# csulb-datascience/TTS-with-Diffusion-model

Measured on NVIDIA B200. Metric: codec_tokens_per_sec, higher is better.
Workload: dtype bf16

## Files before the change

### include/vb200.h

```cpp
#ifndef VB200_H_
#define VB200_H_

#include <stddef.h>
#include <stdint.h>

#ifdef __cplusplus
extern "C" {
#endif

typedef void* vb200_stream_t;

typedef enum {
  VB200_OK = 0,
  VB200_ERR_INVALID = -1,
  VB200_ERR_CUDA = -2,
  VB200_ERR_UNSUPPORTED = -3
} vb200_status;

typedef enum { VB200_F32 = 0, VB200_BF16 = 1, VB200_F16 = 2 } vb200_dtype;

typedef enum {
  VB200_EPI_NONE = 0,
  VB200_EPI_BIAS = 1,
  VB200_EPI_BIAS_GELU = 2,
  VB200_EPI_BIAS_RESIDUAL = 3
} vb200_epilogue;

typedef enum { VB200_ABSORBING = 0, VB200_UNIFORM = 1 } vb200_transition;

typedef enum {
  VB200_NOISE_PHILOX = 0,
  VB200_NOISE_UNIFORMS = 1,
  VB200_NOISE_GREEDY = 2
} vb200_noise;

enum {
  VB200_U_ROW0 = 0,
  VB200_U_TTXT = 1,
  VB200_U_TPROM = 2,
  VB200_U_TRESP = 3,
  VB200_U_TXT0 = 4,
  VB200_U_PROM0 = 5,
  VB200_U_RESP0 = 6,
  VB200_U_GID = 7,
  VB200_U_STRIDE = 8
};

const char* vb200_last_error(void);
int vb200_version(void);
int vb200_device_sms(void);

int vb200_embed_gather(float* x_out, const void* text_w, const void* prom_w, const void* resp_w,
                       const void* sep, const void* time_w, const float* pe,
                       const int32_t* text_ids, const int32_t* prom_ids, const int32_t* resp_ids,
                       const int32_t* utt, const int32_t* row_utt, const int32_t* t_utt,
                       int32_t M, int32_t d, int32_t K, int32_t resp_levels_in,
                       vb200_stream_t stream);


int vb200_adaln(void* out, vb200_dtype out_dtype, const float* x, const float* table, const int32_t* level_utt,
                const int32_t* row_utt, int32_t M, int32_t d, float eps, float k, float c,
                vb200_stream_t stream);

int vb200_layernorm(void* out, vb200_dtype out_dtype, const float* x, const float* weight, const float* bias,
                    int32_t M, int32_t d, float eps, vb200_stream_t stream);

int vb200_gather_rows_bf16(void* out, vb200_dtype out_dtype, const float* x, const int32_t* row_index,
                           int32_t n_rows, int32_t d, vb200_stream_t stream);

int vb200_gemm_bf16(void* out, vb200_dtype out_dtype, const void* A, vb200_dtype a_dtype, const void* W,
                    const float* bias, const float* residual, int32_t M, int32_t N, int32_t K,
                    vb200_epilogue epi, vb200_stream_t stream);

int vb200_gemm_bf16_simt(void* out, vb200_dtype out_dtype, const void* A, vb200_dtype a_dtype, const void* W,
                         const float* bias, const float* residual, int32_t M, int32_t N,
                         int32_t K, vb200_epilogue epi, vb200_stream_t stream);

int vb200_flash_attn_varlen(void* out_bf16, const void* qkv_bf16, const int32_t* cu_rows,
                            int32_t B, int32_t max_T, int32_t M, int32_t n_heads, float scale,
                            vb200_stream_t stream);
int vb200_attn_varlen_simt(void* out_bf16, const void* qkv_bf16, const int32_t* cu_rows,
                           int32_t B, int32_t max_T, int32_t M, int32_t n_heads, float scale,
                           vb200_stream_t stream);

enum {
  VB200_TAB_ONE_KEEP = 0,
  VB200_TAB_ONE_OFF = 1,
  VB200_TAB_ONE_ABSORB = 2,
  VB200_TAB_ONE_BOTH = 3,
  VB200_TAB_CUM_KEEP = 4,
  VB200_TAB_CUM_OFF = 5,
  VB200_TAB_CUM_ABSORB = 6,
  VB200_TAB_CUM_BOTH = 7,
  VB200_TAB_LOG_KEEP = 8,
  VB200_TAB_LOG_OFF = 9,
  VB200_TAB_LOG_ABSORB = 10,
  VB200_TAB_LOG_BOTH = 11,
  VB200_TAB_STRIDE = 12
};

int vb200_q_sample(int32_t* x_out, const int32_t* x0, const int32_t* t_tok, const int32_t* mask,
                   const float* uniforms, const float* table, int32_t n_tok, int32_t K,
                   int32_t S, vb200_transition tr, vb200_stream_t stream);

int vb200_q_sample_dense(int32_t* x_out, const int32_t* x0, const int32_t* t_tok, const int32_t* mask,
                         const float* uniforms, const void* log_qbar_f16, int32_t n_tok, int32_t K,
                         int32_t S, vb200_stream_t stream);

int vb200_q_sample_philox(int32_t* x_out, const int32_t* x0, const int32_t* t_tok, const int32_t* mask,
                          const float* table, int32_t n_tok, int32_t K, int32_t S,
                          vb200_transition tr, uint64_t seed, vb200_stream_t stream);

int vb200_posterior_sample_from_logits(int32_t* x_out, float* post_out, const void* logits,
                                       vb200_dtype logits_dtype, int64_t ld_logits,
                                       const int32_t* x_t, const int32_t* row_utt,
                                       const int32_t* t_utt, const int32_t* utt,
                                       const float* table, int32_t n_rows, int32_t n_levels,
                                       int32_t K, int32_t S, vb200_transition tr,
                                       vb200_noise noise, const float* uniforms, uint64_t seed,
                                       vb200_stream_t stream);

int vb200_head_posterior_sample(int32_t* x_out, void* logits, vb200_dtype logits_dtype,
                                const void* head_in, vb200_dtype head_in_dtype, const void* W,
                                const float* bias, int32_t n_rows, int32_t d, int32_t n_levels, int32_t K,
                                const int32_t* x_t, const int32_t* row_utt, const int32_t* t_utt,
                                const int32_t* utt, const float* table, int32_t S,
                                vb200_transition tr, vb200_noise noise, const float* uniforms,
                                uint64_t seed, vb200_stream_t stream);

int vb200_head_ce_loss(float* loss, const void* head_in, vb200_dtype head_in_dtype, const void* W,
                       const float* bias,
                       const int32_t* targets, int32_t n_rows, int32_t d, int32_t n_levels, int32_t K,
                       vb200_stream_t stream);

int64_t vb200_workspace_bytes(int64_t M, int64_t M_resp, int32_t d, int32_t n_out,
                              vb200_dtype logits_dtype, int64_t* sizes);

int vb200_codes_to_bqt(int64_t* out, const int32_t* codes, const int32_t* utt, int32_t B,
                       int32_t n_levels, int32_t T_max, int64_t pad, vb200_stream_t stream);

int vb200_step_timesteps(int32_t* t_utt, int32_t B, int32_t delta, vb200_stream_t stream);

#ifdef __cplusplus
}
#endif
#endif
```

### tts-with-diffusion-model_b200/csrc/attn_tcgen05.cu

```cuda
#include "common.cuh"
#include <type_traits>

namespace vb200 {

namespace attn {
constexpr int BQ = 128, BKV = 128, HD = 64, KV_STAGES = 2;
constexpr int TILE_BYTES = 128 * HD * 2;
constexpr uint32_t TMEM_COLS = 256;
constexpr uint32_t COL_S = 0, COL_P = 128, COL_O = 192;
constexpr int SOFTMAX_WARPS = 8;
constexpr int THREADS = (SOFTMAX_WARPS + 2) * 32;
constexpr int SMEM_BYTES = TILE_BYTES * (1 + 2 * KV_STAGES) + 1024 + 256;
constexpr float RESCALE_LOG2 = 8.0f;
}

__device__ __forceinline__ void tmem_ld_16x2_x64(uint32_t taddr, uint32_t (&r)[64]) {
  asm volatile(
      "tcgen05.ld.sync.aligned.16x32bx2.x64.b32 "
      "{%0,%1,%2,%3,%4,%5,%6,%7,%8,%9,%10,%11,%12,%13,%14,%15,"
      "%16,%17,%18,%19,%20,%21,%22,%23,%24,%25,%26,%27,%28,%29,%30,%31,"
      "%32,%33,%34,%35,%36,%37,%38,%39,%40,%41,%42,%43,%44,%45,%46,%47,"
      "%48,%49,%50,%51,%52,%53,%54,%55,%56,%57,%58,%59,%60,%61,%62,%63}, [%64], 64;"
      : "=r"(r[0]), "=r"(r[1]), "=r"(r[2]), "=r"(r[3]), "=r"(r[4]), "=r"(r[5]), "=r"(r[6]), "=r"(r[7]),
        "=r"(r[8]), "=r"(r[9]), "=r"(r[10]), "=r"(r[11]), "=r"(r[12]), "=r"(r[13]), "=r"(r[14]), "=r"(r[15]),
        "=r"(r[16]), "=r"(r[17]), "=r"(r[18]), "=r"(r[19]), "=r"(r[20]), "=r"(r[21]), "=r"(r[22]), "=r"(r[23]),
        "=r"(r[24]), "=r"(r[25]), "=r"(r[26]), "=r"(r[27]), "=r"(r[28]), "=r"(r[29]), "=r"(r[30]), "=r"(r[31]),
        "=r"(r[32]), "=r"(r[33]), "=r"(r[34]), "=r"(r[35]), "=r"(r[36]), "=r"(r[37]), "=r"(r[38]), "=r"(r[39]),
        "=r"(r[40]), "=r"(r[41]), "=r"(r[42]), "=r"(r[43]), "=r"(r[44]), "=r"(r[45]), "=r"(r[46]), "=r"(r[47]),
        "=r"(r[48]), "=r"(r[49]), "=r"(r[50]), "=r"(r[51]), "=r"(r[52]), "=r"(r[53]), "=r"(r[54]), "=r"(r[55]),
        "=r"(r[56]), "=r"(r[57]), "=r"(r[58]), "=r"(r[59]), "=r"(r[60]), "=r"(r[61]), "=r"(r[62]), "=r"(r[63])
      : "r"(taddr)
      : "memory");
}
__device__ __forceinline__ void tmem_st_16x2_x32(uint32_t taddr, const uint32_t (&r)[64]) {
  asm volatile(
      "tcgen05.st.sync.aligned.16x32bx2.x32.b32 [%0], 32, "
      "{%1,%2,%3,%4,%5,%6,%7,%8,%9,%10,%11,%12,%13,%14,%15,%16,"
      "%17,%18,%19,%20,%21,%22,%23,%24,%25,%26,%27,%28,%29,%30,%31,%32};"
      ::"r"(taddr), "r"(r[0]), "r"(r[1]), "r"(r[2]), "r"(r[3]), "r"(r[4]), "r"(r[5]), "r"(r[6]), "r"(r[7]),
        "r"(r[8]), "r"(r[9]), "r"(r[10]), "r"(r[11]), "r"(r[12]), "r"(r[13]), "r"(r[14]), "r"(r[15]),
        "r"(r[16]), "r"(r[17]), "r"(r[18]), "r"(r[19]), "r"(r[20]), "r"(r[21]), "r"(r[22]), "r"(r[23]),
        "r"(r[24]), "r"(r[25]), "r"(r[26]), "r"(r[27]), "r"(r[28]), "r"(r[29]), "r"(r[30]), "r"(r[31])
      : "memory");
}
__device__ __forceinline__ void tmem_ld_16x2_x16(uint32_t taddr, uint32_t (&r)[16]) {
  asm volatile(
      "tcgen05.ld.sync.aligned.16x32bx2.x16.b32 "
      "{%0,%1,%2,%3,%4,%5,%6,%7,%8,%9,%10,%11,%12,%13,%14,%15}, [%16], 16;"
      : "=r"(r[0]), "=r"(r[1]), "=r"(r[2]), "=r"(r[3]), "=r"(r[4]), "=r"(r[5]), "=r"(r[6]), "=r"(r[7]),
        "=r"(r[8]), "=r"(r[9]), "=r"(r[10]), "=r"(r[11]), "=r"(r[12]), "=r"(r[13]), "=r"(r[14]), "=r"(r[15])
      : "r"(taddr)
      : "memory");
}
__device__ __forceinline__ void tmem_st_16x2_x16(uint32_t taddr, const uint32_t (&r)[16]) {
  asm volatile(
      "tcgen05.st.sync.aligned.16x32bx2.x16.b32 [%0], 16, "
      "{%1,%2,%3,%4,%5,%6,%7,%8,%9,%10,%11,%12,%13,%14,%15,%16};"
      ::"r"(taddr), "r"(r[0]), "r"(r[1]), "r"(r[2]), "r"(r[3]), "r"(r[4]), "r"(r[5]), "r"(r[6]), "r"(r[7]),
        "r"(r[8]), "r"(r[9]), "r"(r[10]), "r"(r[11]), "r"(r[12]), "r"(r[13]), "r"(r[14]), "r"(r[15])
      : "memory");
}
__device__ __forceinline__ void tmem_st_16x2_x8(uint32_t taddr, const uint32_t (&r)[8]) {
  asm volatile(
      "tcgen05.st.sync.aligned.16x32bx2.x8.b32 [%0], 8, {%1,%2,%3,%4,%5,%6,%7,%8};"
      ::"r"(taddr), "r"(r[0]), "r"(r[1]), "r"(r[2]), "r"(r[3]), "r"(r[4]), "r"(r[5]), "r"(r[6]), "r"(r[7])
      : "memory");
}
__device__ __forceinline__ void tmem_ld_16x2_x32(uint32_t taddr, uint32_t (&r)[32]) {
  asm volatile(
      "tcgen05.ld.sync.aligned.16x32bx2.x32.b32 "
      "{%0,%1,%2,%3,%4,%5,%6,%7,%8,%9,%10,%11,%12,%13,%14,%15,"
      "%16,%17,%18,%19,%20,%21,%22,%23,%24,%25,%26,%27,%28,%29,%30,%31}, [%32], 32;"
      : "=r"(r[0]), "=r"(r[1]), "=r"(r[2]), "=r"(r[3]), "=r"(r[4]), "=r"(r[5]), "=r"(r[6]), "=r"(r[7]),
        "=r"(r[8]), "=r"(r[9]), "=r"(r[10]), "=r"(r[11]), "=r"(r[12]), "=r"(r[13]), "=r"(r[14]), "=r"(r[15]),
        "=r"(r[16]), "=r"(r[17]), "=r"(r[18]), "=r"(r[19]), "=r"(r[20]), "=r"(r[21]), "=r"(r[22]), "=r"(r[23]),
        "=r"(r[24]), "=r"(r[25]), "=r"(r[26]), "=r"(r[27]), "=r"(r[28]), "=r"(r[29]), "=r"(r[30]), "=r"(r[31])
      : "r"(taddr)
      : "memory");
}

__device__ __forceinline__ float ex2_approx(float x) {
  float y;
  asm("ex2.approx.ftz.f32 %0, %1;" : "=f"(y) : "f"(x));
  return y;
}

__device__ __forceinline__ void ex2_poly2(uint64_t x, float& p0, float& p1) {
  float x0, x1;
  unpack2(x, x0, x1);
  x = pack2(fmaxf(x0, -126.0f), fmaxf(x1, -126.0f));
  const uint64_t t = fadd2(x, pack2(12582912.0f, 12582912.0f));
  const uint64_t u = fadd2(t, pack2(-12582912.0f, -12582912.0f));
  const uint64_t r = ffma2(u, pack2(-1.0f, -1.0f), x);
  uint64_t p = ffma2(r, pack2(0.05517167f, 0.05517167f), pack2(0.24261113f, 0.24261113f));
  p = ffma2(r, p, pack2(0.69326097f, 0.69326097f));
  p = ffma2(r, p, pack2(0.99992806f, 0.99992806f));
  float t0, t1, q0, q1;
  unpack2(t, t0, t1);
  unpack2(p, q0, q1);
  p0 = __int_as_float(__float_as_int(q0) + (__float_as_int(t0) << 23));
  p1 = __int_as_float(__float_as_int(q1) + (__float_as_int(t1) << 23));
}
#ifndef VB200_ATTN_EMU_PAIRS
#define VB200_ATTN_EMU_PAIRS 4
#endif
#ifndef VB200_ATTN_EXP_CHUNK
#define VB200_ATTN_EXP_CHUNK 4
#endif
namespace attn { constexpr int EXP_CHUNK = VB200_ATTN_EXP_CHUNK; }

#ifdef VB200_ATTN_TRACE
constexpr int TRACE_CTAS = 1024, TRACE_BLOCKS = 16, TRACE_EVENTS = 8;
__device__ unsigned long long g_attn_trace[TRACE_CTAS * 2 * TRACE_BLOCKS * TRACE_EVENTS];
#define VB_TR(slot, j, ev)                                                                               \
  do {                                                                                                   \
    if (lane == 0 && cta_lin < TRACE_CTAS && (j) < TRACE_BLOCKS)                                         \
      g_attn_trace[((cta_lin * 2 + (slot)) * TRACE_BLOCKS + (j)) * TRACE_EVENTS + (ev)] = clock64();     \
  } while (0)
#else
#define VB_TR(slot, j, ev) do {} while (0)
#endif

__global__ void __launch_bounds__(attn::THREADS, 2) flash_attn_kernel(
    const __grid_constant__ CUtensorMap tm_qkv, __nv_bfloat16* __restrict__ out,
    const int32_t* __restrict__ cu_rows, int n_heads, float scale_log2, float opaque_zero) {
  using namespace attn;
  const int b = blockIdx.z, h = blockIdx.y, qt = blockIdx.x;
  const int row0 = cu_rows[b];
  const int T = cu_rows[b + 1] - row0;
  if (qt * BQ >= T) return;
  const int nblk = (T + BKV - 1) / BKV;
  const int last_valid = T - (nblk - 1) * BKV;
  const int last_n = (last_valid + 15) & ~15;
  const int d = n_heads * HD;

  extern __shared__ uint8_t smem_raw[];
  const uint32_t raw_addr = smem_u32(smem_raw);
  uint8_t* smem = smem_raw + (((raw_addr + 1023u) & ~1023u) - raw_addr);
  uint8_t* s_q = smem;
  uint8_t* s_k = smem + TILE_BYTES;
  uint8_t* s_v = s_k + KV_STAGES * TILE_BYTES;
  uint64_t* bars = reinterpret_cast<uint64_t*>(s_v + KV_STAGES * TILE_BYTES);
  uint64_t* q_full = bars;
  uint64_t* k_full = bars + 1;
  uint64_t* k_empty = k_full + KV_STAGES;
  uint64_t* v_full = k_empty + KV_STAGES;
  uint64_t* v_empty = v_full + KV_STAGES;
  uint64_t* s_full = v_empty + KV_STAGES;
  uint64_t* s_free = s_full + 1;
  uint64_t* p_full = s_free + 1;
  uint64_t* pv_done = p_full + 1;
  uint32_t* tmem_slot = reinterpret_cast<uint32_t*>(pv_done + 1);

  const int warp = __shfl_sync(0xffffffffu, threadIdx.x >> 5, 0);
  const int lane = threadIdx.x & 31;
#ifdef VB200_ATTN_TRACE
  const int cta_lin = blockIdx.x + gridDim.x * (blockIdx.y + gridDim.y * blockIdx.z);
  if (threadIdx.x == 0 && cta_lin < TRACE_CTAS) {
    uint32_t smid;
    asm volatile("mov.u32 %0, %%smid;" : "=r"(smid));
    g_attn_trace[((cta_lin * 2 + 1) * TRACE_BLOCKS + TRACE_BLOCKS - 1) * TRACE_EVENTS + 7] = smid;
    g_attn_trace[((cta_lin * 2 + 1) * TRACE_BLOCKS + TRACE_BLOCKS - 1) * TRACE_EVENTS + 6] = clock64();
  }
#endif

  if (threadIdx.x == SOFTMAX_WARPS * 32) {
    tma_prefetch_desc(&tm_qkv);
    mbar_init(q_full, 1);
    for (int s = 0; s < KV_STAGES; ++s) {
      mbar_init(&k_full[s], 1); mbar_init(&k_empty[s], 1); mbar_init(&v_full[s], 1); mbar_init(&v_empty[s], 1);
    }
    mbar_init(s_full, 1); mbar_init(s_free, SOFTMAX_WARPS); mbar_init(p_full, SOFTMAX_WARPS); mbar_init(pv_done, 1);
    fence_barrier_init();
    pdl_launch_dependents();
    pdl_wait();
    mbar_arrive_expect_tx(q_full, TILE_BYTES);
    tma_load_2d(s_q, &tm_qkv, q_full, h * HD, row0 + qt * BQ);
    mbar_arrive_expect_tx(&k_full[0], TILE_BYTES);
    tma_load_2d(s_k, &tm_qkv, &k_full[0], d + h * HD, row0);
    mbar_arrive_expect_tx(&v_full[0], TILE_BYTES);
    tma_load_2d(s_v, &tm_qkv, &v_full[0], 2 * d + h * HD, row0);
  }
  if (warp == SOFTMAX_WARPS + 1) {
    tmem_alloc(tmem_slot, TMEM_COLS);
    tmem_relinquish();
  }
  tc_fence_before();
  __syncthreads();
  tc_fence_after();
  const uint32_t tmem_base = *tmem_slot;
  pdl_launch_dependents();
  pdl_wait();

  if (warp == SOFTMAX_WARPS) {
    const bool leader = elect_one();
    for (int j = 1; j < nblk; ++j) {
      const int s = j % KV_STAGES;
      const uint32_t ph = (j / KV_STAGES) & 1;
      mbar_wait(&k_empty[s], ph ^ 1);
      if (leader) {
        mbar_arrive_expect_tx(&k_full[s], TILE_BYTES);
        tma_load_2d(s_k + s * TILE_BYTES, &tm_qkv, &k_full[s], d + h * HD, row0 + j * BKV);
      }
      __syncwarp();
      mbar_wait(&v_empty[s], ph ^ 1);
      if (leader) {
        mbar_arrive_expect_tx(&v_full[s], TILE_BYTES);
        tma_load_2d(s_v + s * TILE_BYTES, &tm_qkv, &v_full[s], 2 * d + h * HD, row0 + j * BKV);
      }
      __syncwarp();
    }
  } else if (warp == SOFTMAX_WARPS + 1) {
    const bool leader = elect_one();
    const uint32_t idesc_o = umma_idesc_bf16(BQ, HD, false, true);
    const uint32_t idesc_s_full = umma_idesc_bf16(BQ, BKV, false, false);
    const uint32_t idesc_s_last = umma_idesc_bf16(BQ, last_n, false, false);
    const uint64_t dq = umma_desc_kmajor_sw128(smem_u32(s_q));
    const uint64_t dk_base = umma_desc_kmajor_sw128(smem_u32(s_k));
    const uint64_t dv_base = umma_desc_mnmajor_sw128(smem_u32(s_v), 1024);
    constexpr uint32_t kTileStep = TILE_BYTES >> 4;
    const uint32_t t_s = tmem_base + COL_S, t_p = tmem_base + COL_P, t_o = tmem_base + COL_O;
    auto issue_s = [&](int j) {
      const int st = j % KV_STAGES;
      const uint64_t dk = dk_base + static_cast<uint32_t>(st) * kTileStep;
      const uint32_t idesc_s = (j == nblk - 1) ? idesc_s_last : idesc_s_full;
      if (leader) {
#pragma unroll
        for (int k = 0; k < HD / 16; ++k) umma_ss(t_s, dq + 2 * k, dk + 2 * k, idesc_s, k != 0);
        umma_commit(s_full);
        umma_commit(&k_empty[st]);
      }
      __syncwarp();
    };
    auto issue_pv = [&](int j) {
      const int st = j % KV_STAGES;
      const uint64_t dv = dv_base + static_cast<uint32_t>(st) * kTileStep;
      const uint32_t acc0 = j != 0;
      if (leader) {
        if (j != nblk - 1) {
#pragma unroll
          for (int k = 0; k < BKV / 16; ++k)
            umma_ts(t_o, t_p + k * 8, dv + k * 128, idesc_o, acc0 | (k != 0));
        } else {
          const int ksteps = last_n / 16;
          for (int k = 0; k < ksteps; ++k) umma_ts(t_o, t_p + k * 8, dv + k * 128, idesc_o, acc0 | (k != 0));
        }
        umma_commit(pv_done);
        umma_commit(&v_empty[st]);
      }
      __syncwarp();
    };
    mbar_wait(q_full, 0);
    mbar_wait(&k_full[0], 0);
    tc_fence_after();
    issue_s(0);
    for (int j = 0; j < nblk; ++j) {
      if (j + 1 < nblk) {
        mbar_wait(&k_full[(j + 1) % KV_STAGES], ((j + 1) / KV_STAGES) & 1);
        mbar_wait(s_free, j & 1);
        tc_fence_after();
        VB_TR(1, j, 0);
        issue_s(j + 1);
      }
      mbar_wait(&v_full[j % KV_STAGES], (j / KV_STAGES) & 1);
      mbar_wait(p_full, j & 1);
      tc_fence_after();
      VB_TR(1, j, 1);
      issue_pv(j);
    }
  } else {
    const int quad = warp & 3;
    const int half_rows = warp >> 2;
    const int t0 = lane & 15, t1 = lane >> 4;
    const int r_tile = quad * 32 + half_rows * 16 + t0;
    const uint32_t t_x = tmem_base + (static_cast<uint32_t>(quad * 32 + half_rows * 16) << 16);
    if (qt * BQ + quad * 32 + half_rows * 16 >= T) {
      for (int j = 0; j < nblk; ++j) {
        mbar_wait(s_full, j & 1);
        if (lane == 0) mbar_arrive(s_free);
        if (j > 0) mbar_wait(pv_done, (j - 1) & 1);
        if (lane == 0) mbar_arrive(p_full);
      }
      mbar_wait(pv_done, (nblk - 1) & 1);
    } else {
      float m_ref = -INFINITY, l = 0.f;
      const uint64_t zero2 = pack2(opaque_zero, opaque_zero);
      auto move_reference = [&](float bm, int j) {
        if (j == 0) {
          m_ref = bm;
          return;
        }
        const bool grow = (bm - m_ref) * scale_log2 > RESCALE_LOG2;
        if (__any_sync(0xffffffffu, grow)) {
          const float m_new = grow ? bm : m_ref;
          const float alpha = ex2_approx((m_ref - m_new) * scale_log2);
          m_ref = m_new;
          l *= alpha;
          mbar_wait(pv_done, (j - 1) & 1);
          tc_fence_after();
#pragma unroll 1
          for (int c = 0; c < 2; ++c) {
            uint32_t o[16];
            tmem_ld_16x2_x16(t_x + COL_O + c * 32, o);
            tmem_ld_wait();
#pragma unroll
            for (int i = 0; i < 16; ++i) o[i] = __float_as_uint(__uint_as_float(o[i]) * alpha);
            tmem_st_16x2_x16(t_x + COL_O + c * 32, o);
          }
        }
      };
      auto key_block = [&](int j, auto tail_tag) {
        constexpr bool tail = decltype(tail_tag)::value;
        if (warp == 0) VB_TR(0, j, 0);
        mbar_wait(s_full, j & 1);
        tc_fence_after();
        if (warp == 0) VB_TR(0, j, 1);
        uint32_t s[64];
        tmem_ld_16x2_x64(t_x + COL_S, s);
        tmem_ld_wait();
        if (warp == 0) VB_TR(0, j, 2);
        tc_fence_before();
        __syncwarp();
        if (lane == 0) mbar_arrive(s_free);
        if (tail) {
#pragma unroll
          for (int i = 0; i < 64; ++i)
            if (t1 * 64 + i >= last_valid) s[i] = __float_as_uint(-INFINITY);
        }
        float bm0 = -INFINITY, bm1 = -INFINITY, bm2 = -INFINITY, bm3 = -INFINITY;
#pragma unroll
        for (int i = 0; i < 64; i += 4) {
          bm0 = fmaxf(bm0, __uint_as_float(s[i]));     bm1 = fmaxf(bm1, __uint_as_float(s[i + 1]));
          bm2 = fmaxf(bm2, __uint_as_float(s[i + 2])); bm3 = fmaxf(bm3, __uint_as_float(s[i + 3]));
        }
        float bm = fmaxf(fmaxf(bm0, bm1), fmaxf(bm2, bm3));
        bm = fmaxf(bm, __shfl_xor_sync(0xffffffffu, bm, 16));
        move_reference(bm, j);
        const float mneg = -m_ref * scale_log2;
#ifdef VB200_ATTN_TRACE
        if (warp == 0 && mneg != 12345.f) VB_TR(0, j, 3);
#endif
        const uint64_t scale2 = pack2(scale_log2, scale_log2), mneg2 = pack2(mneg, mneg);
        uint64_t ps[2] = {0ull, 0ull};
#pragma unroll
        for (int k = 0; k < 32 / EXP_CHUNK; ++k) {
          const uint64_t mn2 = k >= 2 ? ffma2(ps[k & 1], zero2, mneg2) : mneg2;
#pragma unroll
          for (int i = k * EXP_CHUNK; i < (k + 1) * EXP_CHUNK; ++i) {
            const uint64_t x = ffma2(pack2(__uint_as_float(s[2 * i]), __uint_as_float(s[2 * i + 1])), scale2, mn2);
            const int ii = i & 15;
            const bool emulate = ((ii + 1) * VB200_ATTN_EMU_PAIRS) / 16 != (ii * VB200_ATTN_EMU_PAIRS) / 16;
            float p0, p1;
            if (emulate) {
              ex2_poly2(x, p0, p1);
            } else {
              float x0, x1;
              unpack2(x, x0, x1);
              p0 = ex2_approx(x0);
              p1 = ex2_approx(x1);
            }
            ps[k & 1] = fadd2(ps[k & 1], pack2(p0, p1));
            s[i] = pack_bf16x2(p0, p1);
          }
        }
        float a0, a1, a2, a3;
        unpack2(ps[0], a0, a1);
        unpack2(ps[1], a2, a3);
        l += (a0 + a1) + (a2 + a3);
#ifdef VB200_ATTN_TRACE
        if (warp == 0 && l != -1.f) VB_TR(0, j, 4);
#endif
        if (j > 0) {
          mbar_wait(pv_done, (j - 1) & 1);
          tc_fence_after();
        }
        if (warp == 0) VB_TR(0, j, 5);
        tmem_st_16x2_x32(t_x + COL_P, s);
        tmem_st_wait();
        tc_fence_before();
        __syncwarp();
        if (lane == 0) mbar_arrive(p_full);
        if (warp == 0) VB_TR(0, j, 6);
      };
      auto short_block = [&](int j) {
        mbar_wait(s_full, j & 1);
        tc_fence_after();
        uint32_t sq[16];
        tmem_ld_16x2_x16(t_x + COL_S, sq);
        tmem_ld_wait();
        tc_fence_before();
        __syncwarp();
        if (lane == 0) mbar_arrive(s_free);
        float bm = -INFINITY;
#pragma unroll
        for (int i = 0; i < 16; ++i) {
          if (t1 * 16 + i >= last_valid) sq[i] = __float_as_uint(-INFINITY);
          bm = fmaxf(bm, __uint_as_float(sq[i]));
        }
        bm = fmaxf(bm, __shfl_xor_sync(0xffffffffu, bm, 16));
        move_reference(bm, j);
        const float mneg = -m_ref * scale_log2;
        uint32_t pq[8];
#pragma unroll
        for (int i = 0; i < 8; ++i) {
          const float p0 = ex2_approx(fmaf(__uint_as_float(sq[2 * i]), scale_log2, mneg));
          const float p1 = ex2_approx(fmaf(__uint_as_float(sq[2 * i + 1]), scale_log2, mneg));
          l += p0 + p1;
          pq[i] = pack_bf16x2(p0, p1);
        }
        if (j > 0) {
          mbar_wait(pv_done, (j - 1) & 1);
          tc_fence_after();
        }
        tmem_st_16x2_x8(t_x + COL_P, pq);
        tmem_st_wait();
        tc_fence_before();
        __syncwarp();
        if (lane == 0) mbar_arrive(p_full);
      };
      const int n_full = last_valid < BKV ? nblk - 1 : nblk;
#pragma unroll 1
      for (int j = 0; j < n_full; ++j) key_block(j, std::false_type{});
      if (n_full < nblk) {
        if (last_valid <= 32) short_block(n_full);
        else key_block(n_full, std::true_type{});
      }
      mbar_wait(pv_done, (nblk - 1) & 1);
      tc_fence_after();
      l += __shfl_xor_sync(0xffffffffu, l, 16);
      uint32_t o[32];
      tmem_ld_16x2_x32(t_x + COL_O, o);
      tmem_ld_wait();
      const int q_row = qt * BQ + r_tile;
      if (q_row < T) {
        const float inv = 1.0f / l;
        __nv_bfloat16* o_dst = out + static_cast<size_t>(row0 + q_row) * d + h * HD + t1 * 32;
#pragma unroll
        for (int i = 0; i < 32; i += 8) {
          uint4 pk;
          pk.x = pack_bf16x2(__uint_as_float(o[i]) * inv, __uint_as_float(o[i + 1]) * inv);
          pk.y = pack_bf16x2(__uint_as_float(o[i + 2]) * inv, __uint_as_float(o[i + 3]) * inv);
          pk.z = pack_bf16x2(__uint_as_float(o[i + 4]) * inv, __uint_as_float(o[i + 5]) * inv);
          pk.w = pack_bf16x2(__uint_as_float(o[i + 6]) * inv, __uint_as_float(o[i + 7]) * inv);
          *reinterpret_cast<uint4*>(o_dst + i) = pk;
        }
      }
    }
  }

  tc_fence_before();
  __syncthreads();
  if (warp == SOFTMAX_WARPS + 1) {
    __syncwarp();
    tc_fence_after();
    tmem_dealloc(tmem_base, TMEM_COLS);
  }
}

}

using namespace vb200;

#ifdef VB200_ATTN_TRACE
extern "C" int vb200_debug_attn_trace(unsigned long long* host_dst, size_t n_words) {
  const size_t n = sizeof(g_attn_trace) / sizeof(unsigned long long);
  cudaError_t e = cudaMemcpyFromSymbol(host_dst, g_attn_trace, (n_words < n ? n_words : n) * sizeof(unsigned long long));
  return e == cudaSuccess ? 0 : -1;
}
#endif

extern "C" int vb200_flash_attn_varlen(void* out_bf16, const void* qkv_bf16, const int32_t* cu_rows,
                                       int32_t B, int32_t max_T, int32_t M, int32_t n_heads,
                                       float scale, vb200_stream_t stream) {
  using namespace attn;
  if (M == 0) return VB200_OK;
  VB_REQUIRE(out_bf16 && qkv_bf16 && cu_rows, "flash_attn: null pointer");
  VB_REQUIRE(B >= 1 && B <= 65535 && n_heads >= 1 && n_heads <= 65535 && max_T >= 1 && M >= 0,
             "flash_attn: bad sizes B=%d heads=%d max_T=%d M=%d", B, n_heads, max_T, M);
  const int d = n_heads * HD;
  CUtensorMap tm;
  int rc = cached_tmap(&tm, VB200_BF16, qkv_bf16, static_cast<uint64_t>(3) * d, M,
                       static_cast<uint64_t>(3) * d * 2, HD, 128);
  if (rc != VB200_OK) return rc;
  dim3 grid((max_T + BQ - 1) / BQ, n_heads, B);
  const float sl2 = scale * 1.4426950408889634f;
  constexpr int SMEM_SOLO = 116 * 1024;
  const bool solo = static_cast<long long>(grid.x) * grid.y * grid.z <= num_sms();
  const int smem_bytes = solo ? SMEM_SOLO : SMEM_BYTES;
  VB_CONFIGURE_SMEM(flash_attn_kernel, SMEM_SOLO);
  {
    static std::atomic<uint64_t> carveout_done{0};
    int dev = 0;
    VB_CHECK_CUDA(cudaGetDevice(&dev));
    const uint64_t bit = 1ull << (dev & 63);
    if (!(carveout_done.load(std::memory_order_acquire) & bit)) {
      VB_CHECK_CUDA(cudaFuncSetAttribute(flash_attn_kernel, cudaFuncAttributePreferredSharedMemoryCarveout,
                                         cudaSharedmemCarveoutMaxShared));
      carveout_done.fetch_or(bit, std::memory_order_release);
    }
  }
  PdlTag pdl_tag(solo ? 16 : 64);
  VB_CHECK_CUDA(launch_pdl(flash_attn_kernel, grid, dim3(THREADS), smem_bytes, static_cast<cudaStream_t>(stream), 1,
                           tm, static_cast<__nv_bfloat16*>(out_bf16), cu_rows, n_heads, sl2, 0.0f));
  VB_CHECK_CUDA(cudaGetLastError());
  return VB200_OK;
}
```

### tts-with-diffusion-model_b200/csrc/common.cuh

```cuda
#pragma once
#include <atomic>
#include <cuda.h>
#include <cuda_bf16.h>
#include <cuda_fp16.h>
#include <cuda_runtime.h>
#include <stdint.h>

#include "../../include/vb200.h"

namespace vb200 {

void set_error(const char* fmt, ...);
int cuda_fail(cudaError_t e, const char* what);
#define VB_CHECK_CUDA(expr)                                              \
  do {                                                                   \
    cudaError_t _e = (expr);                                             \
    if (_e != cudaSuccess) return ::vb200::cuda_fail(_e, #expr);         \
  } while (0)
#define VB_REQUIRE(cond, ...)                                            \
  do {                                                                   \
    if (!(cond)) {                                                       \
      ::vb200::set_error(__VA_ARGS__);                                   \
      return VB200_ERR_INVALID;                                          \
    }                                                                    \
  } while (0)

int num_sms();

bool head_sample_supported(int d, int K, int noise);
int head_sample_fused(int32_t* x_out, const void* head_in, const void* W, const float* bias, const int32_t* x_t,
                      const int32_t* row_utt, const int32_t* t_utt, const int32_t* utt, const float* table,
                      int n_rows, int d, int n_levels, int K, int S, int tr, int noise, uint64_t seed,
                      int in_f16, cudaStream_t st);
int head_ce_fused(float* loss_out, const void* head_in, const void* W, const float* bias, const int32_t* targets,
                  int n_rows, int d, int n_levels, int K, int in_f16, cudaStream_t st);

#define VB_CONFIGURE_SMEM(kern, bytes)                                                                   \
  do {                                                                                                   \
    static std::atomic<uint64_t> vb_cfg_done{0};                                                         \
    int vb_cfg_dev = 0;                                                                                  \
    VB_CHECK_CUDA(cudaGetDevice(&vb_cfg_dev));                                                           \
    const uint64_t vb_cfg_bit = 1ull << (vb_cfg_dev & 63);                                               \
    if (!(vb_cfg_done.load(std::memory_order_acquire) & vb_cfg_bit)) {                                   \
      VB_CHECK_CUDA(cudaFuncSetAttribute(kern, cudaFuncAttributeMaxDynamicSharedMemorySize, bytes));     \
      vb_cfg_done.fetch_or(vb_cfg_bit, std::memory_order_release);                                       \
    }                                                                                                    \
  } while (0)
bool pdl_enabled();
int pdl_mask();
extern thread_local int g_pdl_tag;
struct PdlTag {
  int prev;
  explicit PdlTag(int t) : prev(g_pdl_tag) { g_pdl_tag = t; }
  ~PdlTag() { g_pdl_tag = prev; }
};
template <typename... KArgs, typename... Args>
inline cudaError_t launch_pdl(void (*kern)(KArgs...), dim3 grid, dim3 block, size_t smem, cudaStream_t st,
                              int cluster_x, Args&&... args) {
  cudaLaunchConfig_t cfg = {};
  cfg.gridDim = grid;
  cfg.blockDim = block;
  cfg.dynamicSmemBytes = smem;
  cfg.stream = st;
  cudaLaunchAttribute attr[2];
  int n = 0;
  if (cluster_x > 1) {
    attr[n].id = cudaLaunchAttributeClusterDimension;
    attr[n].val.clusterDim.x = cluster_x;
    attr[n].val.clusterDim.y = 1;
    attr[n].val.clusterDim.z = 1;
    ++n;
  }
  if (pdl_mask() & (1 | g_pdl_tag)) {
    attr[n].id = cudaLaunchAttributeProgrammaticStreamSerialization;
    attr[n].val.programmaticStreamSerializationAllowed = 1;
    ++n;
  }
  cfg.attrs = attr;
  cfg.numAttrs = n;
  return cudaLaunchKernelEx(&cfg, kern, static_cast<KArgs>(args)...);
}

int make_tmap_2d(CUtensorMap* out, vb200_dtype dtype, const void* gptr, uint64_t inner,
                 uint64_t outer, uint64_t row_stride_bytes, uint32_t box_inner, uint32_t box_outer);
int cached_tmap(CUtensorMap* out, vb200_dtype dtype, const void* ptr, uint64_t inner,
                uint64_t outer, uint64_t stride_bytes, uint32_t box_inner, uint32_t box_outer);

__device__ __forceinline__ void pdl_launch_dependents() { asm volatile("griddepcontrol.launch_dependents;"); }
__device__ __forceinline__ void pdl_wait() { asm volatile("griddepcontrol.wait;" ::: "memory"); }

#ifdef __CUDACC__

__device__ __forceinline__ uint32_t smem_u32(const void* p) {
  return static_cast<uint32_t>(__cvta_generic_to_shared(p));
}

__device__ __forceinline__ bool elect_one() {
  uint32_t pred = 0;
  asm volatile(
      "{\n\t.reg .pred P;\n\t"
      "elect.sync _|P, 0xffffffff;\n\t"
      "selp.b32 %0, 1, 0, P;\n\t}"
      : "=r"(pred));
  return pred != 0;
}

__device__ __forceinline__ void mbar_init(uint64_t* bar, uint32_t count) {
  asm volatile("mbarrier.init.shared::cta.b64 [%0], %1;" ::"r"(smem_u32(bar)), "r"(count));
}
__device__ __forceinline__ void fence_barrier_init() {
  asm volatile("fence.mbarrier_init.release.cluster;" ::: "memory");
}
__device__ __forceinline__ void fence_proxy_async_smem() {
  asm volatile("fence.proxy.async.shared::cta;" ::: "memory");
}
__device__ __forceinline__ void mbar_arrive_expect_tx(uint64_t* bar, uint32_t bytes) {
  asm volatile("mbarrier.arrive.expect_tx.shared::cta.b64 _, [%0], %1;" ::"r"(smem_u32(bar)),
               "r"(bytes)
               : "memory");
}
__device__ __forceinline__ void mbar_arrive(uint64_t* bar) {
  asm volatile("mbarrier.arrive.shared::cta.b64 _, [%0];" ::"r"(smem_u32(bar)) : "memory");
}
__device__ __forceinline__ bool mbar_try_wait(uint64_t* bar, uint32_t parity) {
  uint32_t ok;
  asm volatile(
      "{\n\t.reg .pred P;\n\t"
      "mbarrier.try_wait.parity.shared::cta.b64 P, [%1], %2;\n\t"
      "selp.b32 %0, 1, 0, P;\n\t}"
      : "=r"(ok)
      : "r"(smem_u32(bar)), "r"(parity)
      : "memory");
  return ok != 0;
}
__device__ __forceinline__ bool mbar_test_wait(uint64_t* bar, uint32_t parity) {
  uint32_t ok;
  asm volatile(
      "{\n\t.reg .pred P;\n\t"
      "mbarrier.test_wait.parity.shared::cta.b64 P, [%1], %2;\n\t"
      "selp.b32 %0, 1, 0, P;\n\t}"
      : "=r"(ok)
      : "r"(smem_u32(bar)), "r"(parity)
      : "memory");
  return ok != 0;
}
__device__ __forceinline__ void mbar_wait(uint64_t* bar, uint32_t parity) {
  uint32_t spins = 0;
  while (!mbar_try_wait(bar, parity)) {
    if (++spins > (1u << 24)) __trap();
  }
}

__device__ __forceinline__ void prefetch_l1(const void* p) {
  asm volatile("prefetch.global.L1 [%0];" ::"l"(p));
}
__device__ __forceinline__ void tma_prefetch_desc(const CUtensorMap* m) {
  asm volatile("prefetch.tensormap [%0];" ::"l"(reinterpret_cast<uint64_t>(m)) : "memory");
}
__device__ __forceinline__ void tma_load_2d(void* smem_dst, const CUtensorMap* m, uint64_t* bar,
                                            int32_t c_inner, int32_t c_outer) {
  asm volatile(
      "cp.async.bulk.tensor.2d.shared::cluster.global.mbarrier::complete_tx::bytes"
      " [%0], [%1, {%3, %4}], [%2];"
      ::"r"(smem_u32(smem_dst)), "l"(reinterpret_cast<uint64_t>(m)), "r"(smem_u32(bar)),
      "r"(c_inner), "r"(c_outer)
      : "memory");
}

__device__ __forceinline__ void tma_store_2d(const CUtensorMap* m, const void* smem_src,
                                             int32_t c_inner, int32_t c_outer) {
  asm volatile("cp.async.bulk.tensor.2d.global.shared::cta.bulk_group [%0, {%2, %3}], [%1];"
               ::"l"(reinterpret_cast<uint64_t>(m)), "r"(smem_u32(smem_src)), "r"(c_inner),
               "r"(c_outer)
               : "memory");
}
__device__ __forceinline__ void tma_reduce_add_2d(const CUtensorMap* m, const void* smem_src,
                                                  int32_t c_inner, int32_t c_outer) {
  asm volatile("cp.reduce.async.bulk.tensor.2d.global.shared::cta.add.bulk_group [%0, {%2, %3}], [%1];"
               ::"l"(reinterpret_cast<uint64_t>(m)), "r"(smem_u32(smem_src)), "r"(c_inner),
               "r"(c_outer)
               : "memory");
}
__device__ __forceinline__ void tma_store_commit() {
  asm volatile("cp.async.bulk.commit_group;" ::: "memory");
}
__device__ __forceinline__ void tma_store_wait_read() {
  asm volatile("cp.async.bulk.wait_group.read 0;" ::: "memory");
}
__device__ __forceinline__ void tma_store_wait_all() {
  asm volatile("cp.async.bulk.wait_group 0;" ::: "memory");
}

__device__ __forceinline__ void tmem_alloc(uint32_t* smem_slot, uint32_t ncols) {
  asm volatile("tcgen05.alloc.cta_group::1.sync.aligned.shared::cta.b32 [%0], %1;" ::"r"(
                   smem_u32(smem_slot)),
               "r"(ncols)
               : "memory");
}
__device__ __forceinline__ void tmem_relinquish() {
  asm volatile("tcgen05.relinquish_alloc_permit.cta_group::1.sync.aligned;" ::: "memory");
}
__device__ __forceinline__ void tmem_dealloc(uint32_t taddr, uint32_t ncols) {
  asm volatile("tcgen05.dealloc.cta_group::1.sync.aligned.b32 %0, %1;" ::"r"(taddr), "r"(ncols)
               : "memory");
}
__device__ __forceinline__ void tc_fence_before() {
  asm volatile("tcgen05.fence::before_thread_sync;" ::: "memory");
}
__device__ __forceinline__ void tc_fence_after() {
  asm volatile("tcgen05.fence::after_thread_sync;" ::: "memory");
}
__device__ __forceinline__ void umma_ss(uint32_t tmem_d, uint64_t desc_a, uint64_t desc_b,
                                        uint32_t idesc, uint32_t accumulate) {
  asm volatile(
      "{\n\t.reg .pred p;\n\t"
      "setp.ne.b32 p, %4, 0;\n\t"
      "tcgen05.mma.cta_group::1.kind::f16 [%0], %1, %2, %3, p;\n\t}"
      ::"r"(tmem_d), "l"(desc_a), "l"(desc_b), "r"(idesc), "r"(accumulate)
      : "memory");
}
__device__ __forceinline__ void umma_ts(uint32_t tmem_d, uint32_t tmem_a, uint64_t desc_b,
                                        uint32_t idesc, uint32_t accumulate) {
  asm volatile(
      "{\n\t.reg .pred p;\n\t"
      "setp.ne.b32 p, %4, 0;\n\t"
      "tcgen05.mma.cta_group::1.kind::f16 [%0], [%1], %2, %3, p;\n\t}"
      ::"r"(tmem_d), "r"(tmem_a), "l"(desc_b), "r"(idesc), "r"(accumulate)
      : "memory");
}
__device__ __forceinline__ void umma_commit(uint64_t* bar) {
  asm volatile("tcgen05.commit.cta_group::1.mbarrier::arrive::one.shared::cluster.b64 [%0];" ::"r"(
                   smem_u32(bar))
               : "memory");
}
__device__ __forceinline__ void tmem_ld_wait() {
  asm volatile("tcgen05.wait::ld.sync.aligned;" ::: "memory");
}
__device__ __forceinline__ void tmem_st_wait() {
  asm volatile("tcgen05.wait::st.sync.aligned;" ::: "memory");
}
__device__ __forceinline__ void tmem_ld_32x32(uint32_t taddr, uint32_t (&r)[32]) {
  asm volatile(
      "tcgen05.ld.sync.aligned.32x32b.x32.b32 "
      "{%0,%1,%2,%3,%4,%5,%6,%7,%8,%9,%10,%11,%12,%13,%14,%15,"
      "%16,%17,%18,%19,%20,%21,%22,%23,%24,%25,%26,%27,%28,%29,%30,%31}, [%32];"
      : "=r"(r[0]), "=r"(r[1]), "=r"(r[2]), "=r"(r[3]), "=r"(r[4]), "=r"(r[5]), "=r"(r[6]),
        "=r"(r[7]), "=r"(r[8]), "=r"(r[9]), "=r"(r[10]), "=r"(r[11]), "=r"(r[12]), "=r"(r[13]),
        "=r"(r[14]), "=r"(r[15]), "=r"(r[16]), "=r"(r[17]), "=r"(r[18]), "=r"(r[19]),
        "=r"(r[20]), "=r"(r[21]), "=r"(r[22]), "=r"(r[23]), "=r"(r[24]), "=r"(r[25]),
        "=r"(r[26]), "=r"(r[27]), "=r"(r[28]), "=r"(r[29]), "=r"(r[30]), "=r"(r[31])
      : "r"(taddr)
      : "memory");
}
__device__ __forceinline__ void tmem_st_32x32(uint32_t taddr, const uint32_t (&r)[32]) {
  asm volatile(
      "tcgen05.st.sync.aligned.32x32b.x32.b32 [%0], "
      "{%1,%2,%3,%4,%5,%6,%7,%8,%9,%10,%11,%12,%13,%14,%15,%16,"
      "%17,%18,%19,%20,%21,%22,%23,%24,%25,%26,%27,%28,%29,%30,%31,%32};"
      ::"r"(taddr), "r"(r[0]), "r"(r[1]), "r"(r[2]), "r"(r[3]), "r"(r[4]), "r"(r[5]), "r"(r[6]),
      "r"(r[7]), "r"(r[8]), "r"(r[9]), "r"(r[10]), "r"(r[11]), "r"(r[12]), "r"(r[13]),
      "r"(r[14]), "r"(r[15]), "r"(r[16]), "r"(r[17]), "r"(r[18]), "r"(r[19]), "r"(r[20]),
      "r"(r[21]), "r"(r[22]), "r"(r[23]), "r"(r[24]), "r"(r[25]), "r"(r[26]), "r"(r[27]),
      "r"(r[28]), "r"(r[29]), "r"(r[30]), "r"(r[31])
      : "memory");
}

__device__ __forceinline__ uint32_t cluster_ctarank() {
  uint32_t r;
  asm volatile("mov.u32 %0, %%cluster_ctarank;" : "=r"(r));
  return r;
}
__device__ __forceinline__ void cluster_sync_all() {
  asm volatile("barrier.cluster.arrive.release.aligned;" ::: "memory");
  asm volatile("barrier.cluster.wait.acquire.aligned;" ::: "memory");
}
__device__ __forceinline__ void tma_load_2d_pair(void* smem_dst, const CUtensorMap* m, uint64_t* bar,
                                                 int32_t c_inner, int32_t c_outer) {
  asm volatile(
      "cp.async.bulk.tensor.2d.cta_group::2.shared::cluster.global.mbarrier::complete_tx::bytes"
      " [%0], [%1, {%3, %4}], [%2];"
      ::"r"(smem_u32(smem_dst)), "l"(reinterpret_cast<uint64_t>(m)), "r"(smem_u32(bar) & 0xFEFFFFFFu),
      "r"(c_inner), "r"(c_outer)
      : "memory");
}
__device__ __forceinline__ void tmem_alloc_pair(uint32_t* smem_slot, uint32_t ncols) {
  asm volatile("tcgen05.alloc.cta_group::2.sync.aligned.shared::cta.b32 [%0], %1;" ::"r"(
                   smem_u32(smem_slot)),
               "r"(ncols)
               : "memory");
}
__device__ __forceinline__ void tmem_relinquish_pair() {
  asm volatile("tcgen05.relinquish_alloc_permit.cta_group::2.sync.aligned;" ::: "memory");
}
__device__ __forceinline__ void tmem_dealloc_pair(uint32_t taddr, uint32_t ncols) {
  asm volatile("tcgen05.dealloc.cta_group::2.sync.aligned.b32 %0, %1;" ::"r"(taddr), "r"(ncols)
               : "memory");
}
__device__ __forceinline__ void umma_ss_pair(uint32_t tmem_d, uint64_t desc_a, uint64_t desc_b,
                                             uint32_t idesc, uint32_t accumulate) {
  asm volatile(
      "{\n\t.reg .pred p;\n\t"
      "setp.ne.b32 p, %4, 0;\n\t"
      "tcgen05.mma.cta_group::2.kind::f16 [%0], %1, %2, %3, p;\n\t}"
      ::"r"(tmem_d), "l"(desc_a), "l"(desc_b), "r"(idesc), "r"(accumulate)
      : "memory");
}
__device__ __forceinline__ void umma_commit_pair(uint64_t* bar) {
  const uint16_t mask = 3;
  asm volatile(
      "tcgen05.commit.cta_group::2.mbarrier::arrive::one.shared::cluster.multicast::cluster.b64 [%0], %1;"
      ::"r"(smem_u32(bar)), "h"(mask)
      : "memory");
}
__device__ __forceinline__ void mbar_arrive_remote(uint64_t* bar, uint32_t rank) {
  uint32_t remote;
  asm volatile("mapa.shared::cluster.u32 %0, %1, %2;" : "=r"(remote) : "r"(smem_u32(bar)), "r"(rank));
  asm volatile("mbarrier.arrive.release.cluster.shared::cluster.b64 _, [%0];" ::"r"(remote) : "memory");
}

__device__ __forceinline__ uint64_t umma_desc_kmajor_sw128(uint32_t smem_addr) {
  uint64_t d = 0;
  d |= static_cast<uint64_t>((smem_addr & 0x3FFFF) >> 4);
  d |= static_cast<uint64_t>(1) << 16;
  d |= static_cast<uint64_t>(1024 >> 4) << 32;
  d |= static_cast<uint64_t>(1) << 46;
  d |= static_cast<uint64_t>(2) << 61;
  return d;
}
__device__ __forceinline__ uint64_t umma_desc_mnmajor_sw128(uint32_t smem_addr, uint32_t lbo_bytes) {
  uint64_t d = 0;
  d |= static_cast<uint64_t>((smem_addr & 0x3FFFF) >> 4);
  d |= static_cast<uint64_t>((lbo_bytes >> 4) & 0x3FFF) << 16;
  d |= static_cast<uint64_t>(1024 >> 4) << 32;
  d |= static_cast<uint64_t>(1) << 46;
  d |= static_cast<uint64_t>(2) << 61;
  return d;
}
constexpr uint32_t kIdescBf16 = (1u << 7) | (1u << 10);
__host__ __device__ constexpr uint32_t umma_idesc_bf16(uint32_t M, uint32_t N, bool a_mn_major,
                                                       bool b_mn_major) {
  return (1u << 4)
         | kIdescBf16
         | ((a_mn_major ? 1u : 0u) << 15)
         | ((b_mn_major ? 1u : 0u) << 16)
         | ((N >> 3) << 17)
         | ((M >> 4) << 24);
}

__device__ __forceinline__ uint32_t pack_bf16x2(float lo, float hi) {
  __nv_bfloat162 v = __floats2bfloat162_rn(lo, hi);
  return *reinterpret_cast<uint32_t*>(&v);
}
__device__ __forceinline__ uint32_t pack_f16x2(float lo, float hi) {
  uint32_t v;
  asm("cvt.rn.satfinite.f16x2.f32 %0, %1, %2;" : "=r"(v) : "f"(hi), "f"(lo));
  return v;
}
__device__ __forceinline__ uint32_t pack_act16x2(float lo, float hi, bool f16) {
  return f16 ? pack_f16x2(lo, hi) : pack_bf16x2(lo, hi);
}

__device__ __forceinline__ uint64_t pack2(float lo, float hi) {
  uint64_t r;
  asm("mov.b64 %0, {%1, %2};" : "=l"(r) : "f"(lo), "f"(hi));
  return r;
}
__device__ __forceinline__ void unpack2(uint64_t v, float& lo, float& hi) {
  asm("mov.b64 {%0, %1}, %2;" : "=f"(lo), "=f"(hi) : "l"(v));
}
__device__ __forceinline__ uint64_t ffma2(uint64_t a, uint64_t b, uint64_t c) {
  uint64_t d;
  asm("fma.rn.f32x2 %0, %1, %2, %3;" : "=l"(d) : "l"(a), "l"(b), "l"(c));
  return d;
}
__device__ __forceinline__ uint64_t fadd2(uint64_t a, uint64_t b) {
  uint64_t d;
  asm("add.rn.f32x2 %0, %1, %2;" : "=l"(d) : "l"(a), "l"(b));
  return d;
}
constexpr float kEps = 1.0e-6f;

struct Philox {
  uint32_t k0, k1;
  __device__ __forceinline__ uint4 operator()(uint32_t c0, uint32_t c1, uint32_t c2, uint32_t c3) const {
    uint32_t a = k0, b = k1;
#pragma unroll
    for (int r = 0; r < 10; ++r) {
      const uint32_t hi0 = __umulhi(0xD2511F53u, c0), lo0 = 0xD2511F53u * c0;
      const uint32_t hi1 = __umulhi(0xCD9E8D57u, c2), lo1 = 0xCD9E8D57u * c2;
      c0 = hi1 ^ c1 ^ a;
      c1 = lo1;
      c2 = hi0 ^ c3 ^ b;
      c3 = lo0;
      a += 0x9E3779B9u;
      b += 0xBB67AE85u;
    }
    return make_uint4(c0, c1, c2, c3);
  }
};
__device__ __forceinline__ float u01(uint32_t x) { return (x >> 8) * 5.9604644775390625e-8f; }
__device__ __forceinline__ float exp2f_fast(float x) {
  float y;
  asm("ex2.approx.ftz.f32 %0, %1;" : "=f"(y) : "f"(x));
  return y;
}

__device__ __forceinline__ float warp_sum(float v) {
#pragma unroll
  for (int o = 16; o > 0; o >>= 1) v += __shfl_xor_sync(0xffffffffu, v, o);
  return v;
}
__device__ __forceinline__ float warp_max(float v) {
#pragma unroll
  for (int o = 16; o > 0; o >>= 1) v = fmaxf(v, __shfl_xor_sync(0xffffffffu, v, o));
  return v;
}

#endif

template <int NV>
__device__ __forceinline__ void adaln_row_finish(const float (&v)[NV][8], const float (&g)[NV][8],
                                                 const float (&bt)[NV][8], __nv_bfloat16* orow, int lane,
                                                 float eps, float k, float c, bool f16 = false) {
  constexpr int d = NV * 256;
  float s = 0.f;
#pragma unroll
  for (int i = 0; i < NV; ++i)
#pragma unroll
    for (int e = 0; e < 8; ++e) s += v[i][e];
  const float mean = warp_sum(s) * (1.0f / d);
  float q = 0.f;
#pragma unroll
  for (int i = 0; i < NV; ++i)
#pragma unroll
    for (int e = 0; e < 8; ++e) { const float dv = v[i][e] - mean; q += dv * dv; }
  const float rstd = rsqrtf(warp_sum(q) * (1.0f / d) + eps);
#pragma unroll
  for (int i = 0; i < NV; ++i) {
    float y[8];
#pragma unroll
    for (int e = 0; e < 8; ++e) {
      float h = (v[i][e] - mean) * rstd;
      h = c * (1.f - k * h) * h;
      y[e] = fmaf(g[i][e], h, bt[i][e]);
    }
    uint4 o;
    o.x = pack_act16x2(y[0], y[1], f16); o.y = pack_act16x2(y[2], y[3], f16);
    o.z = pack_act16x2(y[4], y[5], f16); o.w = pack_act16x2(y[6], y[7], f16);
    *reinterpret_cast<uint4*>(orow + i * 256 + lane * 8) = o;
  }
}
template <int NV>
__device__ __forceinline__ void adaln_load_params(const float* __restrict__ table, int lvl, int lane,
                                                  float (&g)[NV][8], float (&bt)[NV][8]) {
  constexpr int d = NV * 256;
  const float* gp = table + static_cast<size_t>(lvl) * 2 * d;
#pragma unroll
  for (int i = 0; i < NV; ++i) {
    const float4 g0 = __ldg(reinterpret_cast<const float4*>(gp + i * 256 + lane * 8));
    const float4 g1 = __ldg(reinterpret_cast<const float4*>(gp + i * 256 + lane * 8 + 4));
    const float4 b0 = __ldg(reinterpret_cast<const float4*>(gp + d + i * 256 + lane * 8));
    const float4 b1 = __ldg(reinterpret_cast<const float4*>(gp + d + i * 256 + lane * 8 + 4));
    g[i][0] = g0.x; g[i][1] = g0.y; g[i][2] = g0.z; g[i][3] = g0.w;
    g[i][4] = g1.x; g[i][5] = g1.y; g[i][6] = g1.z; g[i][7] = g1.w;
    bt[i][0] = b0.x; bt[i][1] = b0.y; bt[i][2] = b0.z; bt[i][3] = b0.w;
    bt[i][4] = b1.x; bt[i][5] = b1.y; bt[i][6] = b1.z; bt[i][7] = b1.w;
  }
}

}
```

### tts-with-diffusion-model_b200/csrc/gemm_tcgen05.cu

```cuda
#include <stdlib.h>

#include <type_traits>

#include "common.cuh"

#ifndef VB200_GEMM_BIAS_PREFETCH
#define VB200_GEMM_BIAS_PREFETCH 1
#endif
#ifndef VB200_GEMM_EARLY_LOAD
#define VB200_GEMM_EARLY_LOAD 1
#endif

namespace vb200 {

namespace gemm {
constexpr int BM = 128, BK = 64;
constexpr int A_BYTES = BM * BK * 2;
template <int CTAS, int BN> struct Cfg {
  static constexpr int B_ROWS = BN / CTAS;
  static constexpr int B_BYTES = B_ROWS * BK * 2;
  static constexpr int STAGE_BYTES = A_BYTES + B_BYTES;
  static constexpr int STAGES = (4 * 48 * 1024) / STAGE_BYTES;
};
constexpr int EPI_WARPS = 8;
constexpr int THREADS = (2 + EPI_WARPS) * 32;
constexpr int EPI_TILE_BYTES = 32 * 128;
constexpr int SMEM_BYTES = 4 * 48 * 1024 + EPI_WARPS * EPI_TILE_BYTES + 1024  +
                           256 ;
constexpr uint32_t TMEM_COLS = 512;
}

__device__ __forceinline__ void gelu_erf_fast2(float& x0, float& x1) {
  const float z0 = fminf(fabsf(x0) * 0.70710678118654752f, 6.0f);
  const float z1 = fminf(fabsf(x1) * 0.70710678118654752f, 6.0f);
  const uint64_t z = pack2(z0, z1);
  uint64_t p = ffma2(z, pack2(9.22344479e-05f, 9.22344479e-05f), pack2(-2.20238999e-03f, -2.20238999e-03f));
  p = ffma2(z, p, pack2(2.23510694e-02f, 2.23510694e-02f));
  p = ffma2(z, p, pack2(-1.29628107e-01f, -1.29628107e-01f));
  p = ffma2(z, p, pack2(-9.38564420e-01f, -9.38564420e-01f));
  p = ffma2(z, p, pack2(-1.62045550e+00f, -1.62045550e+00f));
  p = ffma2(z, p, pack2(-1.00044155e+00f, -1.00044155e+00f));
  float p0, p1, q0, q1, h0, h1;
  unpack2(p, p0, p1);
  asm("ex2.approx.ftz.f32 %0, %1;" : "=f"(q0) : "f"(p0));
  asm("ex2.approx.ftz.f32 %0, %1;" : "=f"(q1) : "f"(p1));
  unpack2(ffma2(pack2(q0, q1), pack2(-1.0f, -1.0f), pack2(0.5f, 0.5f)), h0, h1);
  h0 = __uint_as_float(__float_as_uint(h0) | (__float_as_uint(x0) & 0x80000000u));
  h1 = __uint_as_float(__float_as_uint(h1) | (__float_as_uint(x1) & 0x80000000u));
  const uint64_t s = fadd2(pack2(h0, h1), pack2(0.5f, 0.5f));
  unpack2(ffma2(pack2(x0, x1), s, 0ull), x0, x1);
}

template <int EPI, typename OutT, int CTAS, int BN>
__global__ void __launch_bounds__(gemm::THREADS, 1) gemm_tcgen05_kernel(
    const __grid_constant__ CUtensorMap tm_a, const __grid_constant__ CUtensorMap tm_b,
    const __grid_constant__ CUtensorMap tm_out, const float* __restrict__ bias, int M, int N, int K,
    uint32_t a_is_f16) {
  using namespace gemm;
  using C = Cfg<CTAS, BN>;
  constexpr int STAGES = C::STAGES, STAGE_BYTES = C::STAGE_BYTES, B_ROWS = C::B_ROWS;
  constexpr int HALF_COLS = BN / 2;
  const uint32_t cta_rank = CTAS == 2 ? cluster_ctarank() : 0;
  extern __shared__ uint8_t smem_raw[];
  const uint32_t raw_addr = smem_u32(smem_raw);
  const uint32_t pad = ((raw_addr + 1023u) & ~1023u) - raw_addr;
  uint8_t* smem = smem_raw + pad;
  uint8_t* epi_smem = smem + STAGES * STAGE_BYTES;
  uint64_t* bars = reinterpret_cast<uint64_t*>(epi_smem + EPI_WARPS * EPI_TILE_BYTES);
  uint64_t* full = bars;
  uint64_t* empty = bars + STAGES;
  uint64_t* acc_full = bars + 2 * STAGES;
  uint64_t* acc_empty = acc_full + 2;
  uint32_t* tmem_slot = reinterpret_cast<uint32_t*>(acc_empty + 2);

  const int warp = __shfl_sync(0xffffffffu, threadIdx.x >> 5, 0);
  const int lane = threadIdx.x & 31;
  const int num_m = (M + BM * CTAS - 1) / (BM * CTAS), num_n = (N + BN - 1) / BN;
  const int num_tiles = num_m * num_n;
  const int num_kb = (K + BK - 1) / BK;
  const int tile0 = blockIdx.x / CTAS, tile_stride = gridDim.x / CTAS;

  if (threadIdx.x == 0) {
    tma_prefetch_desc(&tm_a);
    tma_prefetch_desc(&tm_b);
    tma_prefetch_desc(&tm_out);
    for (int s = 0; s < STAGES; ++s) { mbar_init(&full[s], 1); mbar_init(&empty[s], 1); }
    for (int a = 0; a < 2; ++a) { mbar_init(&acc_full[a], 1); mbar_init(&acc_empty[a], EPI_WARPS * CTAS); }
    fence_barrier_init();
#if VB200_GEMM_EARLY_LOAD
    if (CTAS == 1 && tile0 < num_tiles) {
      pdl_launch_dependents();
      const int m_row = (tile0 / num_n) * BM, n_row = (tile0 % num_n) * BN;
      const int n_pre = num_kb < STAGES ? num_kb : STAGES;
      for (int kb = 0; kb < n_pre; ++kb) {
        mbar_arrive_expect_tx(&full[kb], STAGE_BYTES);
        tma_load_2d(smem + kb * STAGE_BYTES + A_BYTES, &tm_b, &full[kb], kb * BK, n_row);
      }
      pdl_wait();
      for (int kb = 0; kb < n_pre; ++kb) tma_load_2d(smem + kb * STAGE_BYTES, &tm_a, &full[kb], kb * BK, m_row);
    }
#endif
  }
  if (warp == 1) {
    if (CTAS == 2) { tmem_alloc_pair(tmem_slot, TMEM_COLS); tmem_relinquish_pair(); }
    else { tmem_alloc(tmem_slot, TMEM_COLS); tmem_relinquish(); }
  }
  tc_fence_before();
  if (CTAS == 2) cluster_sync_all(); else __syncthreads();
  tc_fence_after();
  const uint32_t tmem_base = *tmem_slot;
  pdl_launch_dependents();
  pdl_wait();

  if (warp == 0) {
    {
      const bool leader = elect_one();
      int stage = 0; uint32_t phase = 0;
      int kb0 = 0;
#if VB200_GEMM_EARLY_LOAD
      if (CTAS == 1) {
        kb0 = num_kb < STAGES ? num_kb : STAGES;
        if (kb0 == STAGES) phase = 1; else stage = kb0;
      }
#endif
      for (int tile = tile0; tile < num_tiles; tile += tile_stride) {
        const int m_blk = tile / num_n, n_blk = tile % num_n;
        const int m_row = (m_blk * CTAS + cta_rank) * BM, n_row = n_blk * BN + cta_rank * B_ROWS;
        for (int kb = kb0; kb < num_kb; ++kb) {
          mbar_wait(&empty[stage], phase ^ 1);
          uint8_t* sa = smem + stage * STAGE_BYTES;
          if (leader) {
            if (CTAS == 2) {
              if (cta_rank == 0) mbar_arrive_expect_tx(&full[stage], 2 * STAGE_BYTES);
              tma_load_2d_pair(sa, &tm_a, &full[stage], kb * BK, m_row);
              tma_load_2d_pair(sa + A_BYTES, &tm_b, &full[stage], kb * BK, n_row);
            } else {
              mbar_arrive_expect_tx(&full[stage], STAGE_BYTES);
              tma_load_2d(sa, &tm_a, &full[stage], kb * BK, m_row);
              tma_load_2d(sa + A_BYTES, &tm_b, &full[stage], kb * BK, n_row);
            }
          }
          __syncwarp();
          if (++stage == STAGES) { stage = 0; phase ^= 1; }
        }
        kb0 = 0;
      }
    }
  } else if (warp == 1) {
    if (cta_rank == 0) {
      const bool leader = elect_one();
      const uint32_t idesc = umma_idesc_bf16(BM * CTAS, BN, false, false) & ~(a_is_f16 ? kIdescBf16 : 0u);
      int stage = 0; uint32_t phase = 0;
      int it = 0;
      for (int tile = tile0; tile < num_tiles; tile += tile_stride, ++it) {
        const int as = it & 1;
        const uint32_t aphase = (it >> 1) & 1;
        mbar_wait(&acc_empty[as], aphase ^ 1);
        tc_fence_after();
        const uint32_t d_tmem = tmem_base + as * BN;
        for (int kb = 0; kb < num_kb; ++kb) {
          mbar_wait(&full[stage], phase);
          tc_fence_after();
          const uint32_t sa = smem_u32(smem + stage * STAGE_BYTES);
          const uint64_t da = umma_desc_kmajor_sw128(sa);
          const uint64_t db = umma_desc_kmajor_sw128(sa + A_BYTES);
          if (leader) {
#pragma unroll
            for (int k = 0; k < BK / 16; ++k) {
              if (CTAS == 2) umma_ss_pair(d_tmem, da + 2 * k, db + 2 * k, idesc, (kb | k) != 0);
              else umma_ss(d_tmem, da + 2 * k, db + 2 * k, idesc, (kb | k) != 0);
            }
            if (CTAS == 2) umma_commit_pair(&empty[stage]);
            else umma_commit(&empty[stage]);
          }
          __syncwarp();
          if (++stage == STAGES) { stage = 0; phase ^= 1; }
        }
        if (leader) {
          if (CTAS == 2) umma_commit_pair(&acc_full[as]); else umma_commit(&acc_full[as]);
        }
        __syncwarp();
      }
    }
  } else {
    const int e = warp - 2;
    const int quad = warp & 3;
    const int half = e >> 2;
    uint8_t* stage_tile = epi_smem + e * EPI_TILE_BYTES;
    uint8_t* my_row = stage_tile + lane * 128;
    const int sw = lane & 7;
    constexpr bool kWide = sizeof(OutT) == 4;
    constexpr int CHUNK_COLS = kWide ? 32 : 64;
    constexpr int HALF0_COLS = BN == 192 ? 128 : HALF_COLS;
    const int col_base = half * HALF0_COLS;
    const int n_chunks = (half == 0 ? HALF0_COLS : BN - HALF0_COLS) / CHUNK_COLS;
    const bool epi_leader = elect_one();
    int it = 0;
    for (int tile = tile0; tile < num_tiles; tile += tile_stride, ++it) {
      const int m_blk = tile / num_n, n_blk = tile % num_n;
      const int as = it & 1;
      const uint32_t aphase = (it >> 1) & 1;
      if (EPI != VB200_EPI_NONE && VB200_GEMM_BIAS_PREFETCH) {
        const int nb0 = n_blk * BN + col_base + lane * 32;
        if (lane * 32 < n_chunks * CHUNK_COLS && nb0 < N) prefetch_l1(bias + nb0);
      }
      mbar_wait(&acc_full[as], aphase);
      tc_fence_after();
      const int row0 = (m_blk * CTAS + cta_rank) * BM + quad * 32;
      const uint32_t t_row = tmem_base + (static_cast<uint32_t>(quad * 32) << 16) + as * BN + col_base;
#pragma unroll 1
      for (int c = 0; c < n_chunks; ++c) {
        const int n0 = n_blk * BN + col_base + c * CHUNK_COLS;
        if (epi_leader) tma_store_wait_read();
        __syncwarp();
#pragma unroll
        for (int sub = 0; sub < CHUNK_COLS / 32; ++sub) {
          uint32_t r[32];
          tmem_ld_32x32(t_row + c * CHUNK_COLS + sub * 32, r);
          tmem_ld_wait();
          float v[32];
#pragma unroll
          for (int i = 0; i < 32; ++i) v[i] = __uint_as_float(r[i]);
          const int nb = n0 + sub * 32;
          if (EPI != VB200_EPI_NONE) {
            if (nb + 32 <= N) {
#pragma unroll
              for (int i = 0; i < 32; i += 4) {
                const float4 b4 = __ldg(reinterpret_cast<const float4*>(bias + nb + i));
                unpack2(fadd2(pack2(v[i], v[i + 1]), pack2(b4.x, b4.y)), v[i], v[i + 1]);
                unpack2(fadd2(pack2(v[i + 2], v[i + 3]), pack2(b4.z, b4.w)), v[i + 2], v[i + 3]);
              }
            } else {
#pragma unroll
              for (int i = 0; i < 32; ++i) if (nb + i < N) v[i] += __ldg(bias + nb + i);
            }
          }
          if (EPI == VB200_EPI_BIAS_GELU) {
#pragma unroll
            for (int i = 0; i < 32; i += 2) gelu_erf_fast2(v[i], v[i + 1]);
          }
          if (kWide) {
#pragma unroll
            for (int q = 0; q < 8; ++q)
              *reinterpret_cast<float4*>(my_row + ((q ^ sw) << 4)) =
                  make_float4(v[4 * q], v[4 * q + 1], v[4 * q + 2], v[4 * q + 3]);
          } else {
            constexpr bool is_bf16 = std::is_same<OutT, __nv_bfloat16>::value;
#pragma unroll
            for (int q = 0; q < 4; ++q) {
              uint4 p;
              if (is_bf16) {
                p.x = pack_bf16x2(v[8 * q], v[8 * q + 1]); p.y = pack_bf16x2(v[8 * q + 2], v[8 * q + 3]);
                p.z = pack_bf16x2(v[8 * q + 4], v[8 * q + 5]); p.w = pack_bf16x2(v[8 * q + 6], v[8 * q + 7]);
              } else {
                p.x = pack_f16x2(v[8 * q], v[8 * q + 1]); p.y = pack_f16x2(v[8 * q + 2], v[8 * q + 3]);
                p.z = pack_f16x2(v[8 * q + 4], v[8 * q + 5]); p.w = pack_f16x2(v[8 * q + 6], v[8 * q + 7]);
              }
              *reinterpret_cast<uint4*>(my_row + (((sub * 4 + q) ^ sw) << 4)) = p;
            }
          }
        }
        fence_proxy_async_smem();
        __syncwarp();
        if (epi_leader && row0 < M && n0 < N) {
          if (EPI == VB200_EPI_BIAS_RESIDUAL) tma_reduce_add_2d(&tm_out, stage_tile, n0, row0);
          else tma_store_2d(&tm_out, stage_tile, n0, row0);
          tma_store_commit();
        }
      }
      tc_fence_before();
      __syncwarp();
      if (lane == 0) {
        if (CTAS == 2 && cta_rank != 0) mbar_arrive_remote(&acc_empty[as], 0);
        else mbar_arrive(&acc_empty[as]);
      }
    }
    if (epi_leader) tma_store_wait_all();
  }

  tc_fence_before();
  if (CTAS == 2) cluster_sync_all(); else __syncthreads();
  if (warp == 1) {
    __syncwarp();
    tc_fence_after();
    if (CTAS == 2) tmem_dealloc_pair(tmem_base, TMEM_COLS); else tmem_dealloc(tmem_base, TMEM_COLS);
  }
}

template <int EPI, typename OutT>
static int launch_gemm(void* out, vb200_dtype dt, const void* A, vb200_dtype a_dt, const void* W, const float* bias,
                       int M, int N, int K, cudaStream_t st) {
  const uint32_t a_f16 = a_dt == VB200_F16 ? 1u : 0u;
  using namespace gemm;
  PdlTag pdl_tag(EPI == VB200_EPI_BIAS_RESIDUAL ? 8 : 4);
  constexpr int BN = 256;
  const int sms = num_sms(), mt = (M + BM - 1) / BM, nn = (N + BN - 1) / BN;
  const long ksteps = static_cast<long>((K + BK - 1) / BK) * (BK / 16);
  auto waves = [](long tiles, long units) { return (tiles + units - 1) / units; };
  const long t_wide = waves(static_cast<long>(mt) * nn, sms) * ksteps * 163;
  const long t_pair = waves(static_cast<long>((M + 2 * BM - 1) / (2 * BM)) * nn, sms / 2) * ksteps * 135 + 5000;
  const long t_narrow = N > 128 ? waves(static_cast<long>(mt) * ((N + 127) / 128), sms) * ksteps * 99 : (1l << 60);
  const long t_n64 = (sizeof(OutT) == 4 && N > 64) ? waves(static_cast<long>(mt) * ((N + 63) / 64), sms) * ksteps * 75
                                                   : (1l << 60);
  const long tiles_192 = static_cast<long>(mt) * (N / 192);
  const long t_n192 = (sizeof(OutT) == 2 && N % 192 == 0 && tiles_192 <= sms) ? ksteps * 130 : (1l << 60);
  int ctas = t_pair <= t_wide ? 2 : 1;
  bool narrow = false, narrow64 = false, n192 = false;
  long best = ctas == 2 ? t_pair : t_wide;
  if (t_narrow < best) { ctas = 1; narrow = true; best = t_narrow; }
  if (t_n64 < best) { ctas = 1; narrow = false; narrow64 = true; best = t_n64; }
  if (t_n192 < best) { ctas = 1; narrow = false; narrow64 = false; n192 = true; best = t_n192; }
  static int tile_forced = -1;
  if (tile_forced < 0) {
    const char* e = getenv("VB200_GEMM_TILE");
    tile_forced = !e ? 0 : e[0] == 'p' ? 1 : e[0] == 'w' ? 2 : (e[0] == 'n' && e[1] == 'a') ? 3 : (e[0] == 'n' && e[1] == '6') ? 4 : 0;
  }
  if (tile_forced) {
    ctas = tile_forced == 1 ? 2 : 1;
    narrow = tile_forced == 3 && N > 128;
    narrow64 = tile_forced == 4 && sizeof(OutT) == 4 && N > 64;
    n192 = false;
  }
  const int bn = n192 ? 192 : narrow64 ? 64 : (narrow ? 128 : BN);
  CUtensorMap ta, tb, tout;
  int rc = cached_tmap(&ta, a_dt, A, K, M, static_cast<uint64_t>(K) * 2, BK, BM);
  if (rc != VB200_OK) return rc;
  rc = cached_tmap(&tb, a_dt, W, K, N, static_cast<uint64_t>(K) * 2, BK, bn / ctas);
  if (rc != VB200_OK) return rc;
  const int esz = sizeof(OutT);
  rc = cached_tmap(&tout, dt, out, N, M, static_cast<uint64_t>(N) * esz, 128 / esz, 32);
  if (rc != VB200_OK) return rc;
  const int tiles = ((M + BM * ctas - 1) / (BM * ctas)) * ((N + bn - 1) / bn);
  const int groups = num_sms() / ctas;
  const int grid = (tiles < groups ? tiles : groups) * ctas;
  if (n192) {
    if constexpr (sizeof(OutT) == 2) {
      auto kern = gemm_tcgen05_kernel<EPI, OutT, 1, 192>;
      VB_CONFIGURE_SMEM(kern, SMEM_BYTES);
      VB_CHECK_CUDA(launch_pdl(kern, dim3(grid), dim3(THREADS), SMEM_BYTES, st, 1, ta, tb, tout, bias, M, N, K, a_f16));
    }
  } else if (narrow64) {
    if constexpr (sizeof(OutT) == 4) {
      auto kern = gemm_tcgen05_kernel<EPI, OutT, 1, 64>;
      VB_CONFIGURE_SMEM(kern, SMEM_BYTES);
      VB_CHECK_CUDA(launch_pdl(kern, dim3(grid), dim3(THREADS), SMEM_BYTES, st, 1, ta, tb, tout, bias, M, N, K, a_f16));
    }
  } else if (narrow) {
    auto kern = gemm_tcgen05_kernel<EPI, OutT, 1, 128>;
    VB_CONFIGURE_SMEM(kern, SMEM_BYTES);
    VB_CHECK_CUDA(launch_pdl(kern, dim3(grid), dim3(THREADS), SMEM_BYTES, st, 1, ta, tb, tout, bias, M, N, K, a_f16));
  } else if (ctas == 1) {
    auto kern = gemm_tcgen05_kernel<EPI, OutT, 1, 256>;
    VB_CONFIGURE_SMEM(kern, SMEM_BYTES);
    VB_CHECK_CUDA(launch_pdl(kern, dim3(grid), dim3(THREADS), SMEM_BYTES, st, 1, ta, tb, tout, bias, M, N, K, a_f16));
  } else {
    auto kern = gemm_tcgen05_kernel<EPI, OutT, 2, 256>;
    VB_CONFIGURE_SMEM(kern, SMEM_BYTES);
    VB_CHECK_CUDA(launch_pdl(kern, dim3(grid), dim3(THREADS), SMEM_BYTES, st, 2, ta, tb, tout, bias, M, N, K, a_f16));
  }
  VB_CHECK_CUDA(cudaGetLastError());
  return VB200_OK;
}

template <int EPI>
static int launch_gemm_dtype(void* out, vb200_dtype dt, const void* A, vb200_dtype a_dt, const void* W,
                             const float* bias, int M, int N, int K, cudaStream_t st) {
  switch (dt) {
    case VB200_F32: return launch_gemm<EPI, float>(out, dt, A, a_dt, W, bias, M, N, K, st);
    case VB200_BF16: return launch_gemm<EPI, __nv_bfloat16>(out, dt, A, a_dt, W, bias, M, N, K, st);
    case VB200_F16: return launch_gemm<EPI, __half>(out, dt, A, a_dt, W, bias, M, N, K, st);
  }
  set_error("gemm: unknown out dtype %d", static_cast<int>(dt));
  return VB200_ERR_INVALID;
}

}

using namespace vb200;

extern "C" int vb200_gemm_bf16(void* out, vb200_dtype out_dtype, const void* A, vb200_dtype a_dtype, const void* W,
                               const float* bias, const float* residual, int32_t M, int32_t N,
                               int32_t K, vb200_epilogue epi, vb200_stream_t stream) {
  VB_REQUIRE(M >= 0 && N > 0 && K > 0, "gemm: bad sizes M=%d N=%d K=%d", M, N, K);
  VB_REQUIRE(a_dtype == VB200_BF16 || a_dtype == VB200_F16, "gemm: A and W must be bf16 or f16");
  if (M == 0) return VB200_OK;
  VB_REQUIRE(out && A && W, "gemm: null pointer");
  VB_REQUIRE(K % 8 == 0, "gemm: K=%d must be a multiple of 8 (TMA row stride is 16-byte granular)", K);
  VB_REQUIRE(N % 8 == 0, "gemm: N=%d must be a multiple of 8 (16-byte vector stores)", N);
  VB_REQUIRE((reinterpret_cast<uintptr_t>(out) & 15) == 0, "gemm: out must be 16-byte aligned");
  VB_REQUIRE(epi == VB200_EPI_NONE || bias, "gemm: epilogue %d needs bias", static_cast<int>(epi));
  VB_REQUIRE(epi != VB200_EPI_BIAS_RESIDUAL || (residual && out_dtype == VB200_F32),
             "gemm: BIAS_RESIDUAL needs residual and fp32 output");
  cudaStream_t st = static_cast<cudaStream_t>(stream);
  switch (epi) {
    case VB200_EPI_NONE: return launch_gemm_dtype<VB200_EPI_NONE>(out, out_dtype, A, a_dtype, W, bias, M, N, K, st);
    case VB200_EPI_BIAS: return launch_gemm_dtype<VB200_EPI_BIAS>(out, out_dtype, A, a_dtype, W, bias, M, N, K, st);
    case VB200_EPI_BIAS_GELU: return launch_gemm_dtype<VB200_EPI_BIAS_GELU>(out, out_dtype, A, a_dtype, W, bias, M, N, K, st);
    case VB200_EPI_BIAS_RESIDUAL:
      if (residual != static_cast<const float*>(out))
        VB_CHECK_CUDA(cudaMemcpyAsync(out, residual, static_cast<size_t>(M) * N * sizeof(float),
                                      cudaMemcpyDeviceToDevice, st));
      return launch_gemm<VB200_EPI_BIAS_RESIDUAL, float>(out, out_dtype, A, a_dtype, W, bias, M, N, K, st);
  }
  set_error("gemm: unknown epilogue %d", static_cast<int>(epi));
  return VB200_ERR_INVALID;
}
```

### tts-with-diffusion-model_b200/vall_e/b200/engine.py

```python
from __future__ import annotations

import math
import os
from dataclasses import dataclass, field

import numpy as np
import torch

from . import lib as L


def sinusoidal_table(n: int, d_model: int) -> torch.Tensor:
    d_half = d_model // 2
    omega = torch.exp(-math.log(1e4) * (torch.arange(d_half, dtype=torch.float32) / d_half))
    ang = omega[None, :] * torch.arange(n)[:, None]
    return torch.cat([ang.sin(), ang.cos()], dim=-1).contiguous()


def _act_dtypes():
    v = os.environ.get("VB200_ACT", "head")
    on = {"h", "ff", "head"} if v == "f16" else (set() if v == "bf16" else {x.strip() for x in v.split(",")})
    if not on <= {"h", "ff", "head"}:
        raise ValueError(f"VB200_ACT={v!r}: expected f16, bf16 or a comma list of h, ff, head")
    return {k: (torch.float16 if k in on else torch.bfloat16) for k in ("h", "ff", "head")}


ACT = _act_dtypes()


class PackedWeights:

    def __init__(self, sd: dict, n_heads: int, n_layers: int, norm_type: str, device, max_rows: int = 4096):
        dev = torch.device(device)
        if dev.type != "cuda":
            raise L.VB200Error("PackedWeights needs a CUDA device (no CPU fallback)")
        bf = lambda t: t.detach().to(dev, torch.bfloat16).contiguous()
        as_ = lambda t, k: t.detach().to(dev, ACT[k]).contiguous()
        f32 = lambda t: t.detach().to(dev, torch.float32).contiguous()
        self.device = dev
        self.n_heads, self.n_layers, self.norm_type = n_heads, n_layers, norm_type
        self.d = int(sd["sep"].shape[0])
        if self.d % n_heads or self.d // n_heads != 64:
            raise L.VB200Error(f"head_dim must be 64 (d_model={self.d}, n_heads={n_heads})")
        self.text_w = bf(sd["text_emb.weight"])
        self.prom_w = bf(sd["proms_emb.weight"])
        self.resp_w = bf(sd["resps_emb.weight"])
        self.K = int(self.prom_w.shape[1])
        if int(self.resp_w.shape[1]) != self.K:
            raise L.VB200Error("resps_emb and proms_emb must have the same number of classes")
        self.sep = bf(sd["sep"])
        self.time_w = bf(sd["time_emb.weight"]) if "time_emb.weight" in sd else None
        self.layers = []
        for i in range(n_layers):
            p = f"blocks.{i}"
            ly = dict(
                w_qkv=as_(sd[f"{p}.attn.block.to_qkv.weight"], "h"),
                w_out=bf(sd[f"{p}.attn.block.to_out.weight"]),
                b_out=f32(sd[f"{p}.attn.block.to_out.bias"]),
                w_ff1=as_(sd[f"{p}.ffn.block.0.weight"], "h"), b_ff1=f32(sd[f"{p}.ffn.block.0.bias"]),
                w_ff2=as_(sd[f"{p}.ffn.block.3.weight"], "ff"), b_ff2=f32(sd[f"{p}.ffn.block.3.bias"]),
            )
            for which in ("attn", "ffn"):
                if norm_type == "adaln":
                    emb = sd[f"{p}.{which}.norm.emb.weight"].detach().float()
                    logg, beta = emb.chunk(2, dim=-1)
                    ly[f"norm_{which}"] = f32(torch.cat([logg.exp(), beta], dim=-1))
                else:
                    ly[f"norm_{which}"] = (f32(sd[f"{p}.{which}.norm.weight"]), f32(sd[f"{p}.{which}.norm.bias"]))
            self.layers.append(ly)
        self.w_cls = as_(sd["classifier.weight"], "head")
        self.b_cls = f32(sd["classifier.bias"])
        self.n_out = int(self.w_cls.shape[0])
        self._pe, self._pe_retired = None, []
        self.ensure_pe(max_rows)

    def ensure_pe(self, n: int) -> torch.Tensor:
        if self._pe is None or self._pe.shape[0] < n:
            if self._pe is not None:
                self._pe_retired.append(self._pe)
            self._pe = sinusoidal_table(max(n, 1), self.d).to(self.device)
        return self._pe


def check_ids(ids: torch.Tensor, n: int, what: str, lo: int = 0) -> None:
    if ids.numel() == 0 or os.environ.get("VB200_CHECK_IDS", "1")[:1] == "0":
        return
    mn, mx = torch.aminmax(ids)
    mn, mx = int(mn), int(mx)
    if mn < lo or mx >= n:
        raise IndexError(f"{what}: ids must lie in [{lo}, {n}), got [{mn}, {mx}]")


class BatchLayout:

    def __init__(self, text_list, proms_list, resp_lens, device, gids=None, n_text: int | None = None,
                 n_codes: int | None = None):
        dev = torch.device(device)
        B = len(text_list)
        if B == 0:
            raise ValueError("empty batch")
        if not (len(proms_list) == B and len(resp_lens) == B):
            raise ValueError("text_list, proms_list and resps must have the same length")
        t_txt = [int(t.shape[0]) for t in text_list]
        t_prom = [int(p.shape[0]) for p in proms_list]
        t_resp = [int(r) for r in resp_lens]
        for p in proms_list:
            if p.dim() != 2 or p.shape[1] != 8:
                raise ValueError(f"prompts must be (t, 8) code grids, got {tuple(p.shape)}")
        rows = [a + 1 + b + 1 + c for a, b, c in zip(t_txt, t_prom, t_resp)]
        cu = np.zeros(B + 1, dtype=np.int64)
        cu[1:] = np.cumsum(rows)
        if cu[-1] >= 2 ** 31:
            raise ValueError("batch too large for int32 row indices")
        self.B, self.M, self.max_T = B, int(cu[-1]), int(max(rows))
        self.t_txt, self.t_prom, self.t_resp, self.rows = t_txt, t_prom, t_resp, rows
        self.M_resp = int(sum(t_resp))
        utt = np.zeros((B, L.U_STRIDE), dtype=np.int32)
        utt[:, L.U_ROW0] = cu[:-1]
        utt[:, L.U_TTXT], utt[:, L.U_TPROM], utt[:, L.U_TRESP] = t_txt, t_prom, t_resp
        utt[:, L.U_TXT0] = np.concatenate([[0], np.cumsum(t_txt)[:-1]])
        utt[:, L.U_PROM0] = np.concatenate([[0], np.cumsum(t_prom)[:-1]])
        resp0 = np.concatenate([[0], np.cumsum(t_resp)[:-1]])
        utt[:, L.U_RESP0] = resp0
        utt[:, L.U_GID] = np.arange(B) if gids is None else np.asarray(gids)
        row_utt = np.repeat(np.arange(B, dtype=np.int32), rows)
        resp_row_utt = np.repeat(np.arange(B, dtype=np.int32), t_resp)
        resp_row_index = np.concatenate(
            [np.arange(cu[b + 1] - t_resp[b], cu[b + 1], dtype=np.int32) for b in range(B)]
        ) if self.M_resp else np.zeros(0, dtype=np.int32)
        self.resp_offsets = resp0.tolist()

        def up(a):
            return torch.from_numpy(np.ascontiguousarray(a)).pin_memory().to(dev, non_blocking=True)

        self.utt, self.row_utt, self.cu_rows = up(utt), up(row_utt), up(cu.astype(np.int32))
        self.resp_row_utt, self.resp_row_index = up(resp_row_utt), up(resp_row_index)
        text = torch.cat([t.reshape(-1) for t in text_list]).to(torch.int32)
        proms = torch.cat([p.reshape(-1, 8) for p in proms_list]).to(torch.int32)
        self.n_text, self.n_codes = n_text, n_codes
        if n_text is not None:
            check_ids(text, n_text, "text_list")
        if n_codes is not None:
            check_ids(proms, n_codes, "proms_list")
        self.text_ids = text.contiguous().to(dev, non_blocking=True)
        self.prom_ids = proms.contiguous().to(dev, non_blocking=True)
        self.h2d_bytes = int(utt.nbytes + row_utt.nbytes + (B + 1) * 4 + resp_row_utt.nbytes +
                             resp_row_index.nbytes + text.numel() * 4 + proms.numel() * 4)
        self.device = dev

    def split_resp(self, packed: torch.Tensor):
        return list(packed.split(self.t_resp, dim=0))


@dataclass
class Workspace:
    x: torch.Tensor
    h: torch.Tensor
    qkv: torch.Tensor
    att: torch.Tensor
    ff: torch.Tensor
    head_in: torch.Tensor
    logits: torch.Tensor
    extra: dict = field(default_factory=dict)


class DenoiserEngine:

    def __init__(self, weights: PackedWeights, logits_dtype=torch.float16, attn_variant="tmem", simt=False):
        self.w = weights
        self.logits_dtype = logits_dtype
        self.attn_variant = attn_variant
        self.simt = simt
        self.launches = 0
        self.profile = None

    def workspace(self, lay: BatchLayout, logits_dtype=None) -> Workspace:
        w, dev = self.w, self.w.device
        d, M, Mr = w.d, lay.M, lay.M_resp
        e = lambda *s, dt: torch.empty(*s, dtype=dt, device=dev)
        w.ensure_pe(lay.max_T)
        ldt = logits_dtype or self.logits_dtype
        total, sizes = L.workspace_bytes(M, Mr, d, w.n_out, ldt)
        flat = e(max(total, 1), dt=torch.uint8)
        shapes = {"x": ((M, d), torch.float32), "h": ((M, d), ACT["h"]), "qkv": ((M, 3 * d), torch.bfloat16),
                  "att": ((M, d), torch.bfloat16), "ff": ((M, 4 * d), ACT["ff"]),
                  "head_in": ((Mr, d), ACT["head"]), "logits": ((Mr, w.n_out), ldt)}
        views, off = {}, 0
        for name, size in zip(L.WS_FIELDS, sizes):
            shape, dt = shapes[name]
            n = shape[0] * shape[1] * torch.empty((), dtype=dt).element_size()
            views[name] = flat[off:off + n].view(dt).view(shape)
            off += size
        return Workspace(extra={"flat": flat}, **views)

    def forward(self, lay: BatchLayout, ws: Workspace, resp_ids: torch.Tensor, level_utt: torch.Tensor,
                use_time: bool, hidden_out: list | None = None, head: bool = True) -> torch.Tensor:
        with torch.cuda.device(self.w.device):
            return self._forward(lay, ws, resp_ids, level_utt, use_time, hidden_out, head)

    def _forward(self, lay, ws, resp_ids, level_utt, use_time, hidden_out, head):
        w = self.w
        sv = self.simt
        levels_in = int(resp_ids.shape[1])
        L.embed_gather(ws.x, w.text_w, w.prom_w, w.resp_w, w.sep, w.time_w if use_time else None,
                       w.ensure_pe(lay.max_T), lay.text_ids, lay.prom_ids, resp_ids, lay.utt, lay.row_utt,
                       level_utt, w.K, levels_in)
        scale = 64 ** -0.5
        gemm, attn_flops = self._gemm, sum(4 * T * T * w.d for T in lay.rows)
        for ly in w.layers:
            self._norm(ws.h, ws.x, ly["norm_attn"], level_utt, lay)
            gemm(ws.qkv, ws.h, ly["w_qkv"], epi=L.EPI_NONE)
            ev = self._prof_begin()
            L.flash_attn_varlen(ws.att, ws.qkv, lay.cu_rows, lay.max_T, w.n_heads, scale,
                                variant="simt" if sv else self.attn_variant)
            self._prof_end(ev, "attn", attn_flops)
            gemm(ws.x, ws.att, ly["w_out"], ly["b_out"], residual=ws.x, epi=L.EPI_BIAS_RESIDUAL)
            self._norm(ws.h, ws.x, ly["norm_ffn"], level_utt, lay)
            gemm(ws.ff, ws.h, ly["w_ff1"], ly["b_ff1"], epi=L.EPI_BIAS_GELU)
            gemm(ws.x, ws.ff, ly["w_ff2"], ly["b_ff2"], residual=ws.x, epi=L.EPI_BIAS_RESIDUAL)
            if hidden_out is not None:
                hidden_out.append(ws.x.clone())
        L.gather_rows_bf16(ws.head_in, ws.x, lay.resp_row_index)
        self.launches += 1 + 7 * len(w.layers) + 1
        if not head:
            return ws.head_in
        gemm(ws.logits, ws.head_in, w.w_cls, w.b_cls, epi=L.EPI_BIAS)
        self.launches += 1
        return ws.logits

    def _gemm(self, out, A, W, bias=None, residual=None, epi=L.EPI_NONE):
        ev = self._prof_begin()
        L.gemm_bf16(out, A, W, bias, residual=residual, epi=epi, simt=self.simt)
        self._prof_end(ev, "gemm", 2 * A.shape[0] * A.shape[1] * W.shape[0])

    def _prof_begin(self):
        if self.profile is None:
            return None
        ev = torch.cuda.Event(enable_timing=True)
        ev.record()
        return ev

    def _prof_end(self, ev, kind, flops):
        if ev is None:
            return
        end = torch.cuda.Event(enable_timing=True)
        end.record()
        self.profile.append((kind, flops, ev, end))

    def _norm(self, out, x, params, level_utt, lay):
        ev = self._prof_begin()
        if self.w.norm_type == "adaln":
            L.adaln(out, x, params, level_utt, lay.row_utt)
        else:
            L.layernorm(out, x, params[0], params[1])
        self._prof_end(ev, "norm", x.numel() * 6)

    def session(self, lay: BatchLayout) -> "Session":
        return Session(self, lay)

    def reverse_loop(self, lay: BatchLayout, ws: Workspace, x_t: torch.Tensor, table: torch.Tensor,
                     timesteps: int, transition: int, noise: int = L.NOISE_PHILOX, seed: int = 0,
                     uniforms_fn=None, use_graph: bool = True, n_levels: int = 8, trace: list | None = None):
        ses = Session(self, lay, ws=ws, x_t=x_t)
        ses.run(table, timesteps, transition, noise=noise, seed=seed, uniforms_fn=uniforms_fn,
                use_graph=use_graph, n_levels=n_levels, trace=trace)
        return x_t


class Session:

    def __init__(self, engine: DenoiserEngine, lay: BatchLayout, ws: Workspace | None = None,
                 x_t: torch.Tensor | None = None, n_levels: int = 8):
        self.eng, self.lay = engine, lay
        dev = engine.w.device
        self.ws = ws if ws is not None else engine.workspace(lay)
        self.x_t = x_t if x_t is not None else torch.empty(lay.M_resp, n_levels, dtype=torch.int32, device=dev)
        self.t_utt = torch.zeros(lay.B, dtype=torch.int32, device=dev)
        self.graph = None
        self.graph_key = None
        self.per_step_launches = 0

    def signature(self):
        return (tuple(self.lay.t_txt), tuple(self.lay.t_prom), tuple(self.lay.t_resp))

    def load(self, text_list, proms_list, gids=None) -> int:
        lay = self.lay
        if [len(t) for t in text_list] != lay.t_txt or [len(p) for p in proms_list] != lay.t_prom:
            raise ValueError("batch shape does not match this session")
        text = torch.cat([t.reshape(-1) for t in text_list]).to(torch.int32)
        proms = torch.cat([p.reshape(-1, 8) for p in proms_list]).to(torch.int32)
        if lay.n_text is not None:
            check_ids(text, lay.n_text, "text_list")
        if lay.n_codes is not None:
            check_ids(proms, lay.n_codes, "proms_list")
        lay.text_ids.copy_(text, non_blocking=True)
        lay.prom_ids.copy_(proms, non_blocking=True)
        moved = (text.numel() + proms.numel()) * 4
        if gids is not None:
            g = torch.as_tensor(gids, dtype=torch.int32)
            lay.utt[:, L.U_GID].copy_(g, non_blocking=True)
            moved += g.numel() * 4
        return moved

    def run(self, table: torch.Tensor, timesteps: int, transition: int, noise: int = L.NOISE_PHILOX,
            seed: int = 0, uniforms_fn=None, use_graph: bool = True, n_levels: int = 8,
            trace: list | None = None) -> torch.Tensor:
        with torch.cuda.device(self.eng.w.device):
            return self._run(table, timesteps, transition, noise, seed, uniforms_fn, use_graph, n_levels, trace)

    def _run(self, table, timesteps, transition, noise, seed, uniforms_fn, use_graph, n_levels, trace):
        eng, lay, ws, x_t, t_utt = self.eng, self.lay, self.ws, self.x_t, self.t_utt
        w, dev = eng.w, eng.w.device
        K = w.n_out // n_levels
        t_utt.fill_(timesteps - 1)

        def one_step(uniforms=None):
            if eng.profile is None and not eng.simt:
                head_in = eng._forward(lay, ws, x_t, t_utt, True, None, False)
                L.head_posterior_sample(x_t, ws.logits, head_in, w.w_cls, w.b_cls, x_t, lay.resp_row_utt, t_utt,
                                        lay.utt, table, n_levels, K, transition, noise, uniforms, seed)
                eng.launches += 0 if L.head_fused(w.d, K, noise) else 1
            else:
                logits = eng._forward(lay, ws, x_t, t_utt, True, None, True)
                L.posterior_sample_from_logits(x_t, None, logits, w.n_out, x_t, lay.resp_row_utt, t_utt, lay.utt,
                                               table, lay.M_resp, n_levels, K, transition, noise, uniforms, seed)
            L.step_timesteps(t_utt, -1)
            eng.launches += 2

        n_steps = timesteps - 1
        graph_ok = (use_graph and noise != L.NOISE_UNIFORMS and trace is None and n_steps > 2
                    and eng.profile is None)
        if not graph_ok:
            for t in range(timesteps - 1, 0, -1):
                one_step(uniforms_fn(t) if noise == L.NOISE_UNIFORMS else None)
                if trace is not None:
                    trace.append(x_t.clone())
            return x_t
        key = (table.data_ptr(), transition, noise, seed, n_levels)
        first = 0
        if self.graph is None or self.graph_key != key:
            one_step()
            first = 1
            g = torch.cuda.CUDAGraph()
            cap_stream = torch.cuda.Stream(device=dev)
            cap_stream.wait_stream(torch.cuda.current_stream(dev))
            before = eng.launches
            with torch.cuda.stream(cap_stream):
                with torch.cuda.graph(g, stream=cap_stream):
                    one_step()
            self.per_step_launches = eng.launches - before
            eng.launches = before
            torch.cuda.current_stream(dev).wait_stream(cap_stream)
            self.graph, self.graph_key = g, key
        for _ in range(n_steps - first):
            self.graph.replay()
            eng.launches += self.per_step_launches
        return x_t
```

### tts-with-diffusion-model_b200/vall_e/b200/lib.py

```python
from __future__ import annotations

import ctypes as C
import os
from pathlib import Path

import torch

_HERE = Path(__file__).resolve().parent
LIB_PATH = Path(os.environ.get("VB200_LIB", _HERE / "libvalle_b200.so"))

OK = 0
F32, BF16, F16 = 0, 1, 2
EPI_NONE, EPI_BIAS, EPI_BIAS_GELU, EPI_BIAS_RESIDUAL = 0, 1, 2, 3
ABSORBING, UNIFORM = 0, 1
NOISE_PHILOX, NOISE_UNIFORMS, NOISE_GREEDY = 0, 1, 2
U_ROW0, U_TTXT, U_TPROM, U_TRESP, U_TXT0, U_PROM0, U_RESP0, U_GID, U_STRIDE = range(9)
(TAB_ONE_KEEP, TAB_ONE_OFF, TAB_ONE_ABSORB, TAB_ONE_BOTH, TAB_CUM_KEEP, TAB_CUM_OFF, TAB_CUM_ABSORB,
 TAB_CUM_BOTH, TAB_LOG_KEEP, TAB_LOG_OFF, TAB_LOG_ABSORB, TAB_LOG_BOTH, TAB_STRIDE) = range(13)

_DTYPES = {torch.float32: F32, torch.bfloat16: BF16, torch.float16: F16}

_p, _i32, _i64, _u64, _f = C.c_void_p, C.c_int32, C.c_int64, C.c_uint64, C.c_float

PROTOTYPES = {
    "vb200_last_error": ([], C.c_char_p),
    "vb200_version": ([], C.c_int),
    "vb200_device_sms": ([], C.c_int),
    "vb200_embed_gather": ([_p] * 13 + [_i32] * 4 + [_p], C.c_int),
    "vb200_adaln": ([_p, C.c_int] + [_p] * 4 + [_i32, _i32, _f, _f, _f, _p], C.c_int),
    "vb200_layernorm": ([_p, C.c_int] + [_p] * 3 + [_i32, _i32, _f, _p], C.c_int),
    "vb200_gather_rows_bf16": ([_p, C.c_int, _p, _p, _i32, _i32, _p], C.c_int),
    "vb200_gemm_bf16": ([_p, C.c_int, _p, C.c_int, _p, _p, _p, _i32, _i32, _i32, C.c_int, _p], C.c_int),
    "vb200_gemm_bf16_simt": ([_p, C.c_int, _p, C.c_int, _p, _p, _p, _i32, _i32, _i32, C.c_int, _p], C.c_int),
    "vb200_flash_attn_varlen": ([_p, _p, _p, _i32, _i32, _i32, _i32, _f, _p], C.c_int),
    "vb200_attn_varlen_simt": ([_p, _p, _p, _i32, _i32, _i32, _i32, _f, _p], C.c_int),
    "vb200_q_sample": ([_p] * 6 + [_i32, _i32, _i32, C.c_int, _p], C.c_int),
    "vb200_q_sample_dense": ([_p] * 6 + [_i32, _i32, _i32, _p], C.c_int),
    "vb200_posterior_sample_from_logits": (
        [_p, _p, _p, C.c_int, _i64, _p, _p, _p, _p, _p, _i32, _i32, _i32, _i32, C.c_int, C.c_int, _p, _u64, _p],
        C.c_int),
    "vb200_head_posterior_sample": (
        [_p, _p, C.c_int, _p, C.c_int, _p, _p, _i32, _i32, _i32, _i32, _p, _p, _p, _p, _p, _i32, C.c_int, C.c_int, _p, _u64,
         _p],
        C.c_int),
    "vb200_q_sample_philox": ([_p] * 5 + [_i32, _i32, _i32, C.c_int, _u64, _p], C.c_int),
    "vb200_head_ce_loss": ([_p, _p, C.c_int, _p, _p, _p, _i32, _i32, _i32, _i32, _p], C.c_int),
    "vb200_workspace_bytes": ([_i64, _i64, _i32, _i32, C.c_int, C.POINTER(C.c_int64)], C.c_int64),
    "vb200_step_timesteps": ([_p, _i32, _i32, _p], C.c_int),
    "vb200_codes_to_bqt": ([_p, _p, _p, _i32, _i32, _i32, _i64, _p], C.c_int),
}

_lib = None


class VB200Error(RuntimeError):
    pass


def load() -> C.CDLL:
    global _lib
    if _lib is not None:
        return _lib
    if not LIB_PATH.exists():
        raise VB200Error(
            f"{LIB_PATH} is missing: build it with `python tts-with-diffusion-model_b200/build.py` "
            "(the CUDA library is the only implementation of the hot path; there is no fallback)")
    lib = C.CDLL(str(LIB_PATH))
    for name, (argtypes, restype) in PROTOTYPES.items():
        fn = getattr(lib, name)
        fn.argtypes = argtypes
        fn.restype = restype
    _lib = lib
    return lib


def last_error() -> str:
    return load().vb200_last_error().decode("utf-8", "replace")


def _check(rc: int, what: str) -> None:
    if rc != OK:
        raise VB200Error(f"{what} failed with status {rc}: {last_error()}")


_call_devices: set = set()


def ptr(t: torch.Tensor | None):
    if t is None:
        return None
    if not t.is_cuda or not t.is_contiguous():
        _call_devices.clear()
        raise VB200Error("vb200 kernels take CUDA tensors only (no CPU fallback)" if not t.is_cuda
                         else "vb200 kernels take contiguous tensors")
    _call_devices.add(t.device.index)
    return t.data_ptr()


def stream():
    devs = set(_call_devices)
    _call_devices.clear()
    cur = torch.cuda.current_device()
    if len(devs) > 1:
        raise VB200Error(f"tensors of one call live on different devices: cuda:{sorted(devs)}")
    if devs and devs != {cur}:
        raise VB200Error(f"tensors live on cuda:{devs.pop()} but the current CUDA device is cuda:{cur}; "
                         "wrap the call in `with torch.cuda.device(...)`")
    return torch.cuda.current_stream(cur).cuda_stream


def dtype_code(dt: torch.dtype) -> int:
    return _DTYPES[dt]


def act_code(t: torch.Tensor) -> int:
    if t.dtype not in (torch.bfloat16, torch.float16):
        raise VB200Error(f"16-bit activations must be bf16 or fp16, got {t.dtype}")
    return _DTYPES[t.dtype]


def embed_gather(x_out, text_w, prom_w, resp_w, sep, time_w, pe, text_ids, prom_ids, resp_ids, utt,
                 row_utt, t_utt, K, resp_levels_in):
    M, d = x_out.shape
    _check(load().vb200_embed_gather(ptr(x_out), ptr(text_w), ptr(prom_w), ptr(resp_w), ptr(sep),
                                     ptr(time_w), ptr(pe), ptr(text_ids), ptr(prom_ids), ptr(resp_ids),
                                     ptr(utt), ptr(row_utt), ptr(t_utt), M, d, K, resp_levels_in,
                                     stream()), "vb200_embed_gather")


def adaln(out, x, table, level_utt, row_utt, eps=1e-5, k=0.1, c=2.0):
    M, d = x.shape
    _check(load().vb200_adaln(ptr(out), act_code(out), ptr(x), ptr(table), ptr(level_utt), ptr(row_utt), M, d, eps,
                              k, c, stream()), "vb200_adaln")


def layernorm(out, x, weight, bias, eps=1e-5):
    M, d = x.shape
    _check(load().vb200_layernorm(ptr(out), act_code(out), ptr(x), ptr(weight), ptr(bias), M, d, eps, stream()),
           "vb200_layernorm")


def gather_rows_bf16(out, x, row_index):
    n, d = out.shape
    _check(load().vb200_gather_rows_bf16(ptr(out), act_code(out), ptr(x), ptr(row_index), n, d, stream()),
           "vb200_gather_rows_bf16")


def codes_to_bqt(out, codes, utt, pad=0):
    B, n_levels, T_max = out.shape
    assert out.dtype == torch.int64 and codes.dtype == torch.int32 and out.is_contiguous() and codes.is_contiguous()
    _check(load().vb200_codes_to_bqt(ptr(out), ptr(codes), ptr(utt), B, n_levels, T_max, int(pad), stream()),
           "vb200_codes_to_bqt")


def gemm_bf16(out, A, W, bias=None, residual=None, epi=EPI_NONE, simt=False):
    M, K = A.shape
    N = W.shape[0]
    assert W.shape[1] == K and tuple(out.shape) == (M, N), (A.shape, W.shape, out.shape)
    assert A.dtype in (torch.bfloat16, torch.float16) and W.dtype == A.dtype, (A.dtype, W.dtype)
    fn = load().vb200_gemm_bf16_simt if simt else load().vb200_gemm_bf16
    _check(fn(ptr(out), dtype_code(out.dtype), ptr(A), act_code(A), ptr(W), ptr(bias), ptr(residual), M, N, K, epi,
              stream()), "vb200_gemm_bf16")


def flash_attn_varlen(out, qkv, cu_rows, max_T, n_heads, scale, variant="tmem"):
    M = qkv.shape[0]
    B = cu_rows.numel() - 1
    fn = {"tmem": load().vb200_flash_attn_varlen, "simt": load().vb200_attn_varlen_simt}[variant]
    _check(fn(ptr(out), ptr(qkv), ptr(cu_rows), B, max_T, M, n_heads, scale, stream()),
           f"vb200_flash_attn_varlen[{variant}]")


def q_sample(x_out, x0, t_tok, mask, uniforms, table, K, transition):
    n = x0.numel()
    _check(load().vb200_q_sample(ptr(x_out), ptr(x0), ptr(t_tok), ptr(mask), ptr(uniforms), ptr(table), n, K,
                                 table.shape[0], transition, stream()), "vb200_q_sample")


def q_sample_dense(x_out, x0, t_tok, mask, uniforms, log_qbar):
    S, K, _ = log_qbar.shape
    assert log_qbar.dtype == torch.float16
    _check(load().vb200_q_sample_dense(ptr(x_out), ptr(x0), ptr(t_tok), ptr(mask), ptr(uniforms), ptr(log_qbar),
                                       x0.numel(), K, S, stream()), "vb200_q_sample_dense")


def posterior_sample_from_logits(x_out, post_out, logits, ld_logits, x_t, row_utt, t_utt, utt, table,
                                 n_rows, n_levels, K, transition, noise, uniforms=None, seed=0):
    _check(load().vb200_posterior_sample_from_logits(
        ptr(x_out), ptr(post_out), ptr(logits), dtype_code(logits.dtype), ld_logits, ptr(x_t),
        ptr(row_utt), ptr(t_utt), ptr(utt), ptr(table), n_rows, n_levels, K, table.shape[0], transition,
        noise, ptr(uniforms), seed, stream()), "vb200_posterior_sample_from_logits")


def head_posterior_sample(x_out, logits, head_in, W, bias, x_t, row_utt, t_utt, utt, table, n_levels, K,
                          transition, noise, uniforms=None, seed=0):
    n_rows, d = head_in.shape
    _check(load().vb200_head_posterior_sample(
        ptr(x_out), ptr(logits), dtype_code(logits.dtype) if logits is not None else dtype_code(torch.float16),
        ptr(head_in), act_code(head_in), ptr(W), ptr(bias), n_rows, d,
        n_levels, K, ptr(x_t), ptr(row_utt), ptr(t_utt), ptr(utt), ptr(table), table.shape[0], transition,
        noise, ptr(uniforms), seed, stream()), "vb200_head_posterior_sample")


def q_sample_philox(x_out, x0, t_tok, mask, table, K, transition, seed=0):
    _check(load().vb200_q_sample_philox(ptr(x_out), ptr(x0), ptr(t_tok), ptr(mask), ptr(table), x0.numel(), K,
                                        table.shape[0], transition, seed, stream()), "vb200_q_sample_philox")


def head_ce_loss(loss, head_in, W, bias, targets, n_levels, K):
    n_rows, d = head_in.shape
    _check(load().vb200_head_ce_loss(ptr(loss), ptr(head_in), act_code(head_in), ptr(W), ptr(bias), ptr(targets),
                                     n_rows, d, n_levels, K, stream()), "vb200_head_ce_loss")


def head_fused(d, K, noise) -> bool:
    import os
    return (os.environ.get("VB200_FUSED_HEAD", "1")[:1] != "0" and K % 256 == 0 and 256 <= K <= 4096
            and d % 8 == 0 and noise != NOISE_UNIFORMS)


WS_FIELDS = ("x", "h", "qkv", "att", "ff", "head_in", "logits")


def workspace_bytes(M, M_resp, d, n_out, logits_dtype):
    sizes = (C.c_int64 * 7)()
    total = load().vb200_workspace_bytes(M, M_resp, d, n_out, dtype_code(logits_dtype), sizes)
    if total < 0:
        raise VB200Error(f"vb200_workspace_bytes failed with status {total}: {last_error()}")
    return int(total), [int(v) for v in sizes]


def step_timesteps(t_utt, delta):
    _check(load().vb200_step_timesteps(ptr(t_utt), t_utt.numel(), delta, stream()), "vb200_step_timesteps")
```

Before: 321,400.

## Compute last transformer layer only for response rows and fuse residual into GEMM

In the final layer, after the full QKV projection, attention, out-projection, FFN norm and FFN GEMMs are computed only for the response-token query rows that feed the classifier head. A new attention entry point writes those rows compactly, and a new GEMM epilogue adds a residual gathered through a row index, which also removes the separate gather kernel. Separately, the existing bias+residual path now reads the residual inside the GEMM epilogue instead of issuing a device-to-device memcpy first. The cost is extra epilogue register pressure from residual loads, plus reuse of the qkv buffer as scratch for the float residual stream.

```diff
diff --git a/include/vb200.h b/include/vb200.h
--- a/include/vb200.h
+++ b/include/vb200.h
@@ -72,6 +72,10 @@
                     const float* bias, const float* residual, int32_t M, int32_t N, int32_t K,
                     vb200_epilogue epi, vb200_stream_t stream);
 
+int vb200_gemm_residual_rows(void* out, vb200_dtype out_dtype, const void* A, vb200_dtype a_dtype, const void* W,
+                             const float* bias, const float* residual, const int32_t* residual_rows, int32_t M,
+                             int32_t N, int32_t K, vb200_stream_t stream);
+
 int vb200_gemm_bf16_simt(void* out, vb200_dtype out_dtype, const void* A, vb200_dtype a_dtype, const void* W,
                          const float* bias, const float* residual, int32_t M, int32_t N,
                          int32_t K, vb200_epilogue epi, vb200_stream_t stream);
@@ -79,6 +83,9 @@
 int vb200_flash_attn_varlen(void* out_bf16, const void* qkv_bf16, const int32_t* cu_rows,
                             int32_t B, int32_t max_T, int32_t M, int32_t n_heads, float scale,
                             vb200_stream_t stream);
+int vb200_flash_attn_resp_rows(void* out_bf16, const void* qkv_bf16, const int32_t* cu_rows, const int32_t* utt,
+                               int32_t B, int32_t max_T_resp, int32_t M, int32_t n_heads, float scale,
+                               vb200_stream_t stream);
 int vb200_attn_varlen_simt(void* out_bf16, const void* qkv_bf16, const int32_t* cu_rows,
                            int32_t B, int32_t max_T, int32_t M, int32_t n_heads, float scale,
                            vb200_stream_t stream);
diff --git a/tts-with-diffusion-model_b200/csrc/attn_tcgen05.cu b/tts-with-diffusion-model_b200/csrc/attn_tcgen05.cu
--- a/tts-with-diffusion-model_b200/csrc/attn_tcgen05.cu
+++ b/tts-with-diffusion-model_b200/csrc/attn_tcgen05.cu
@@ -123,12 +123,19 @@
 
 __global__ void __launch_bounds__(attn::THREADS, 2) flash_attn_kernel(
     const __grid_constant__ CUtensorMap tm_qkv, __nv_bfloat16* __restrict__ out,
-    const int32_t* __restrict__ cu_rows, int n_heads, float scale_log2, float opaque_zero) {
+    const int32_t* __restrict__ cu_rows, const int32_t* __restrict__ utt, int n_heads, float scale_log2,
+    float opaque_zero) {
   using namespace attn;
   const int b = blockIdx.z, h = blockIdx.y, qt = blockIdx.x;
   const int row0 = cu_rows[b];
   const int T = cu_rows[b + 1] - row0;
-  if (qt * BQ >= T) return;
+  int n_q = T, q_first = 0, out_row0 = row0;
+  if (utt) {
+    n_q = utt[b * VB200_U_STRIDE + VB200_U_TRESP];
+    q_first = T - n_q;
+    out_row0 = utt[b * VB200_U_STRIDE + VB200_U_RESP0];
+  }
+  if (qt * BQ >= n_q) return;
   const int nblk = (T + BKV - 1) / BKV;
   const int last_valid = T - (nblk - 1) * BKV;
   const int last_n = (last_valid + 15) & ~15;
@@ -175,7 +182,7 @@
     pdl_launch_dependents();
     pdl_wait();
     mbar_arrive_expect_tx(q_full, TILE_BYTES);
-    tma_load_2d(s_q, &tm_qkv, q_full, h * HD, row0 + qt * BQ);
+    tma_load_2d(s_q, &tm_qkv, q_full, h * HD, row0 + q_first + qt * BQ);
     mbar_arrive_expect_tx(&k_full[0], TILE_BYTES);
     tma_load_2d(s_k, &tm_qkv, &k_full[0], d + h * HD, row0);
     mbar_arrive_expect_tx(&v_full[0], TILE_BYTES);
@@ -274,7 +281,7 @@
     const int t0 = lane & 15, t1 = lane >> 4;
     const int r_tile = quad * 32 + half_rows * 16 + t0;
     const uint32_t t_x = tmem_base + (static_cast<uint32_t>(quad * 32 + half_rows * 16) << 16);
-    if (qt * BQ + quad * 32 + half_rows * 16 >= T) {
+    if (qt * BQ + quad * 32 + half_rows * 16 >= n_q) {
       for (int j = 0; j < nblk; ++j) {
         mbar_wait(s_full, j & 1);
         if (lane == 0) mbar_arrive(s_free);
@@ -432,9 +439,9 @@
       tmem_ld_16x2_x32(t_x + COL_O, o);
       tmem_ld_wait();
       const int q_row = qt * BQ + r_tile;
-      if (q_row < T) {
+      if (q_row < n_q) {
         const float inv = 1.0f / l;
-        __nv_bfloat16* o_dst = out + static_cast<size_t>(row0 + q_row) * d + h * HD + t1 * 32;
+        __nv_bfloat16* o_dst = out + static_cast<size_t>(out_row0 + q_row) * d + h * HD + t1 * 32;
 #pragma unroll
         for (int i = 0; i < 32; i += 8) {
           uint4 pk;
@@ -469,20 +476,19 @@
 }
 #endif
 
-extern "C" int vb200_flash_attn_varlen(void* out_bf16, const void* qkv_bf16, const int32_t* cu_rows,
-                                       int32_t B, int32_t max_T, int32_t M, int32_t n_heads,
-                                       float scale, vb200_stream_t stream) {
+static int launch_flash_attn(void* out_bf16, const void* qkv_bf16, const int32_t* cu_rows, const int32_t* utt,
+                             int32_t B, int32_t max_q, int32_t M, int32_t n_heads, float scale, vb200_stream_t stream) {
   using namespace attn;
   if (M == 0) return VB200_OK;
   VB_REQUIRE(out_bf16 && qkv_bf16 && cu_rows, "flash_attn: null pointer");
-  VB_REQUIRE(B >= 1 && B <= 65535 && n_heads >= 1 && n_heads <= 65535 && max_T >= 1 && M >= 0,
-             "flash_attn: bad sizes B=%d heads=%d max_T=%d M=%d", B, n_heads, max_T, M);
+  VB_REQUIRE(B >= 1 && B <= 65535 && n_heads >= 1 && n_heads <= 65535 && max_q >= 1 && M >= 0,
+             "flash_attn: bad sizes B=%d heads=%d max_T=%d M=%d", B, n_heads, max_q, M);
   const int d = n_heads * HD;
   CUtensorMap tm;
   int rc = cached_tmap(&tm, VB200_BF16, qkv_bf16, static_cast<uint64_t>(3) * d, M,
                        static_cast<uint64_t>(3) * d * 2, HD, 128);
   if (rc != VB200_OK) return rc;
-  dim3 grid((max_T + BQ - 1) / BQ, n_heads, B);
+  dim3 grid((max_q + BQ - 1) / BQ, n_heads, B);
   const float sl2 = scale * 1.4426950408889634f;
   constexpr int SMEM_SOLO = 116 * 1024;
   const bool solo = static_cast<long long>(grid.x) * grid.y * grid.z <= num_sms();
@@ -501,7 +507,21 @@
   }
   PdlTag pdl_tag(solo ? 16 : 64);
   VB_CHECK_CUDA(launch_pdl(flash_attn_kernel, grid, dim3(THREADS), smem_bytes, static_cast<cudaStream_t>(stream), 1,
-                           tm, static_cast<__nv_bfloat16*>(out_bf16), cu_rows, n_heads, sl2, 0.0f));
+                           tm, static_cast<__nv_bfloat16*>(out_bf16), cu_rows, utt, n_heads, sl2, 0.0f));
   VB_CHECK_CUDA(cudaGetLastError());
   return VB200_OK;
 }
+
+extern "C" int vb200_flash_attn_varlen(void* out_bf16, const void* qkv_bf16, const int32_t* cu_rows,
+                                       int32_t B, int32_t max_T, int32_t M, int32_t n_heads,
+                                       float scale, vb200_stream_t stream) {
+  return launch_flash_attn(out_bf16, qkv_bf16, cu_rows, nullptr, B, max_T, M, n_heads, scale, stream);
+}
+
+extern "C" int vb200_flash_attn_resp_rows(void* out_bf16, const void* qkv_bf16, const int32_t* cu_rows,
+                                          const int32_t* utt, int32_t B, int32_t max_T_resp, int32_t M,
+                                          int32_t n_heads, float scale, vb200_stream_t stream) {
+  if (max_T_resp == 0) return VB200_OK;
+  VB_REQUIRE(utt || M == 0, "flash_attn_resp_rows: null utt");
+  return launch_flash_attn(out_bf16, qkv_bf16, cu_rows, utt, B, max_T_resp, M, n_heads, scale, stream);
+}
diff --git a/tts-with-diffusion-model_b200/csrc/common.cuh b/tts-with-diffusion-model_b200/csrc/common.cuh
--- a/tts-with-diffusion-model_b200/csrc/common.cuh
+++ b/tts-with-diffusion-model_b200/csrc/common.cuh
@@ -154,6 +154,9 @@
 __device__ __forceinline__ void prefetch_l1(const void* p) {
   asm volatile("prefetch.global.L1 [%0];" ::"l"(p));
 }
+__device__ __forceinline__ void prefetch_l2(const void* p) {
+  asm volatile("prefetch.global.L2 [%0];" ::"l"(p));
+}
 __device__ __forceinline__ void tma_prefetch_desc(const CUtensorMap* m) {
   asm volatile("prefetch.tensormap [%0];" ::"l"(reinterpret_cast<uint64_t>(m)) : "memory");
 }
diff --git a/tts-with-diffusion-model_b200/csrc/gemm_tcgen05.cu b/tts-with-diffusion-model_b200/csrc/gemm_tcgen05.cu
--- a/tts-with-diffusion-model_b200/csrc/gemm_tcgen05.cu
+++ b/tts-with-diffusion-model_b200/csrc/gemm_tcgen05.cu
@@ -14,6 +14,7 @@
 namespace vb200 {
 
 namespace gemm {
+constexpr int EPI_RESIDUAL_ROWS = 4;
 constexpr int BM = 128, BK = 64;
 constexpr int A_BYTES = BM * BK * 2;
 template <int CTAS, int BN> struct Cfg {
@@ -55,7 +56,7 @@
 __global__ void __launch_bounds__(gemm::THREADS, 1) gemm_tcgen05_kernel(
     const __grid_constant__ CUtensorMap tm_a, const __grid_constant__ CUtensorMap tm_b,
     const __grid_constant__ CUtensorMap tm_out, const float* __restrict__ bias, int M, int N, int K,
-    uint32_t a_is_f16) {
+    uint32_t a_is_f16, const float* __restrict__ residual, const int32_t* __restrict__ res_rows) {
   using namespace gemm;
   using C = Cfg<CTAS, BN>;
   constexpr int STAGES = C::STAGES, STAGE_BYTES = C::STAGE_BYTES, B_ROWS = C::B_ROWS;
@@ -191,7 +192,7 @@
     const int sw = lane & 7;
     constexpr bool kWide = sizeof(OutT) == 4;
     constexpr int CHUNK_COLS = kWide ? 32 : 64;
-    constexpr int HALF0_COLS = BN == 192 ? 128 : HALF_COLS;
+    constexpr int HALF0_COLS = BN == 192 ? 128 : (BN == 64 && !kWide) ? 64 : HALF_COLS;
     const int col_base = half * HALF0_COLS;
     const int n_chunks = (half == 0 ? HALF0_COLS : BN - HALF0_COLS) / CHUNK_COLS;
     const bool epi_leader = elect_one();
@@ -204,9 +205,15 @@
         const int nb0 = n_blk * BN + col_base + lane * 32;
         if (lane * 32 < n_chunks * CHUNK_COLS && nb0 < N) prefetch_l1(bias + nb0);
       }
+      const int row0 = (m_blk * CTAS + cta_rank) * BM + quad * 32;
+      const float* res_row = nullptr;
+      if (EPI == EPI_RESIDUAL_ROWS && row0 + lane < M) {
+        res_row = residual + static_cast<size_t>(res_rows ? res_rows[row0 + lane] : row0 + lane) * N;
+        const int nb0 = n_blk * BN + col_base, n_end = min(nb0 + n_chunks * CHUNK_COLS, N);
+        for (int n = nb0; n < n_end; n += 32) prefetch_l2(res_row + n);
+      }
       mbar_wait(&acc_full[as], aphase);
       tc_fence_after();
-      const int row0 = (m_blk * CTAS + cta_rank) * BM + quad * 32;
       const uint32_t t_row = tmem_base + (static_cast<uint32_t>(quad * 32) << 16) + as * BN + col_base;
 #pragma unroll 1
       for (int c = 0; c < n_chunks; ++c) {
@@ -215,13 +222,20 @@
         __syncwarp();
 #pragma unroll
         for (int sub = 0; sub < CHUNK_COLS / 32; ++sub) {
+          const int nb = n0 + sub * 32;
+          float4 res[8];
+          if (EPI == EPI_RESIDUAL_ROWS) {
+#pragma unroll
+            for (int i = 0; i < 8; ++i)
+              res[i] = res_row && nb + 4 * i < N ? __ldg(reinterpret_cast<const float4*>(res_row + nb + 4 * i))
+                                                  : make_float4(0.f, 0.f, 0.f, 0.f);
+          }
           uint32_t r[32];
           tmem_ld_32x32(t_row + c * CHUNK_COLS + sub * 32, r);
           tmem_ld_wait();
           float v[32];
 #pragma unroll
           for (int i = 0; i < 32; ++i) v[i] = __uint_as_float(r[i]);
-          const int nb = n0 + sub * 32;
           if (EPI != VB200_EPI_NONE) {
             if (nb + 32 <= N) {
 #pragma unroll
@@ -238,6 +252,13 @@
           if (EPI == VB200_EPI_BIAS_GELU) {
 #pragma unroll
             for (int i = 0; i < 32; i += 2) gelu_erf_fast2(v[i], v[i + 1]);
+          }
+          if (EPI == EPI_RESIDUAL_ROWS) {
+#pragma unroll
+            for (int i = 0; i < 8; ++i) {
+              unpack2(fadd2(pack2(res[i].x, res[i].y), pack2(v[4 * i], v[4 * i + 1])), v[4 * i], v[4 * i + 1]);
+              unpack2(fadd2(pack2(res[i].z, res[i].w), pack2(v[4 * i + 2], v[4 * i + 3])), v[4 * i + 2], v[4 * i + 3]);
+            }
           }
           if (kWide) {
 #pragma unroll
@@ -289,10 +310,11 @@
 
 template <int EPI, typename OutT>
 static int launch_gemm(void* out, vb200_dtype dt, const void* A, vb200_dtype a_dt, const void* W, const float* bias,
-                       int M, int N, int K, cudaStream_t st) {
+                       int M, int N, int K, cudaStream_t st, const float* residual = nullptr,
+                       const int32_t* res_rows = nullptr) {
   const uint32_t a_f16 = a_dt == VB200_F16 ? 1u : 0u;
   using namespace gemm;
-  PdlTag pdl_tag(EPI == VB200_EPI_BIAS_RESIDUAL ? 8 : 4);
+  PdlTag pdl_tag(EPI == VB200_EPI_BIAS_RESIDUAL || EPI == EPI_RESIDUAL_ROWS ? 8 : 4);
   constexpr int BN = 256;
   const int sms = num_sms(), mt = (M + BM - 1) / BM, nn = (N + BN - 1) / BN;
   const long ksteps = static_cast<long>((K + BK - 1) / BK) * (BK / 16);
@@ -300,8 +322,8 @@
   const long t_wide = waves(static_cast<long>(mt) * nn, sms) * ksteps * 163;
   const long t_pair = waves(static_cast<long>((M + 2 * BM - 1) / (2 * BM)) * nn, sms / 2) * ksteps * 135 + 5000;
   const long t_narrow = N > 128 ? waves(static_cast<long>(mt) * ((N + 127) / 128), sms) * ksteps * 99 : (1l << 60);
-  const long t_n64 = (sizeof(OutT) == 4 && N > 64) ? waves(static_cast<long>(mt) * ((N + 63) / 64), sms) * ksteps * 75
-                                                   : (1l << 60);
+  constexpr bool kN64 = sizeof(OutT) == 4 || EPI == EPI_RESIDUAL_ROWS;
+  const long t_n64 = (kN64 && N > 64) ? waves(static_cast<long>(mt) * ((N + 63) / 64), sms) * ksteps * 75 : (1l << 60);
   const long tiles_192 = static_cast<long>(mt) * (N / 192);
   const long t_n192 = (sizeof(OutT) == 2 && N % 192 == 0 && tiles_192 <= sms) ? ksteps * 130 : (1l << 60);
   int ctas = t_pair <= t_wide ? 2 : 1;
@@ -318,7 +340,7 @@
   if (tile_forced) {
     ctas = tile_forced == 1 ? 2 : 1;
     narrow = tile_forced == 3 && N > 128;
-    narrow64 = tile_forced == 4 && sizeof(OutT) == 4 && N > 64;
+    narrow64 = tile_forced == 4 && kN64 && N > 64;
     n192 = false;
   }
   const int bn = n192 ? 192 : narrow64 ? 64 : (narrow ? 128 : BN);
@@ -337,26 +359,26 @@
     if constexpr (sizeof(OutT) == 2) {
       auto kern = gemm_tcgen05_kernel<EPI, OutT, 1, 192>;
       VB_CONFIGURE_SMEM(kern, SMEM_BYTES);
-      VB_CHECK_CUDA(launch_pdl(kern, dim3(grid), dim3(THREADS), SMEM_BYTES, st, 1, ta, tb, tout, bias, M, N, K, a_f16));
+      VB_CHECK_CUDA(launch_pdl(kern, dim3(grid), dim3(THREADS), SMEM_BYTES, st, 1, ta, tb, tout, bias, M, N, K, a_f16, residual, res_rows));
     }
   } else if (narrow64) {
-    if constexpr (sizeof(OutT) == 4) {
+    if constexpr (kN64) {
       auto kern = gemm_tcgen05_kernel<EPI, OutT, 1, 64>;
       VB_CONFIGURE_SMEM(kern, SMEM_BYTES);
-      VB_CHECK_CUDA(launch_pdl(kern, dim3(grid), dim3(THREADS), SMEM_BYTES, st, 1, ta, tb, tout, bias, M, N, K, a_f16));
+      VB_CHECK_CUDA(launch_pdl(kern, dim3(grid), dim3(THREADS), SMEM_BYTES, st, 1, ta, tb, tout, bias, M, N, K, a_f16, residual, res_rows));
     }
   } else if (narrow) {
     auto kern = gemm_tcgen05_kernel<EPI, OutT, 1, 128>;
     VB_CONFIGURE_SMEM(kern, SMEM_BYTES);
-    VB_CHECK_CUDA(launch_pdl(kern, dim3(grid), dim3(THREADS), SMEM_BYTES, st, 1, ta, tb, tout, bias, M, N, K, a_f16));
+    VB_CHECK_CUDA(launch_pdl(kern, dim3(grid), dim3(THREADS), SMEM_BYTES, st, 1, ta, tb, tout, bias, M, N, K, a_f16, residual, res_rows));
   } else if (ctas == 1) {
     auto kern = gemm_tcgen05_kernel<EPI, OutT, 1, 256>;
     VB_CONFIGURE_SMEM(kern, SMEM_BYTES);
-    VB_CHECK_CUDA(launch_pdl(kern, dim3(grid), dim3(THREADS), SMEM_BYTES, st, 1, ta, tb, tout, bias, M, N, K, a_f16));
+    VB_CHECK_CUDA(launch_pdl(kern, dim3(grid), dim3(THREADS), SMEM_BYTES, st, 1, ta, tb, tout, bias, M, N, K, a_f16, residual, res_rows));
   } else {
     auto kern = gemm_tcgen05_kernel<EPI, OutT, 2, 256>;
     VB_CONFIGURE_SMEM(kern, SMEM_BYTES);
-    VB_CHECK_CUDA(launch_pdl(kern, dim3(grid), dim3(THREADS), SMEM_BYTES, st, 2, ta, tb, tout, bias, M, N, K, a_f16));
+    VB_CHECK_CUDA(launch_pdl(kern, dim3(grid), dim3(THREADS), SMEM_BYTES, st, 2, ta, tb, tout, bias, M, N, K, a_f16, residual, res_rows));
   }
   VB_CHECK_CUDA(cudaGetLastError());
   return VB200_OK;
@@ -364,11 +386,12 @@
 
 template <int EPI>
 static int launch_gemm_dtype(void* out, vb200_dtype dt, const void* A, vb200_dtype a_dt, const void* W,
-                             const float* bias, int M, int N, int K, cudaStream_t st) {
+                             const float* bias, int M, int N, int K, cudaStream_t st,
+                             const float* residual = nullptr, const int32_t* res_rows = nullptr) {
   switch (dt) {
-    case VB200_F32: return launch_gemm<EPI, float>(out, dt, A, a_dt, W, bias, M, N, K, st);
-    case VB200_BF16: return launch_gemm<EPI, __nv_bfloat16>(out, dt, A, a_dt, W, bias, M, N, K, st);
-    case VB200_F16: return launch_gemm<EPI, __half>(out, dt, A, a_dt, W, bias, M, N, K, st);
+    case VB200_F32: return launch_gemm<EPI, float>(out, dt, A, a_dt, W, bias, M, N, K, st, residual, res_rows);
+    case VB200_BF16: return launch_gemm<EPI, __nv_bfloat16>(out, dt, A, a_dt, W, bias, M, N, K, st, residual, res_rows);
+    case VB200_F16: return launch_gemm<EPI, __half>(out, dt, A, a_dt, W, bias, M, N, K, st, residual, res_rows);
   }
   set_error("gemm: unknown out dtype %d", static_cast<int>(dt));
   return VB200_ERR_INVALID;
@@ -397,11 +420,29 @@
     case VB200_EPI_BIAS: return launch_gemm_dtype<VB200_EPI_BIAS>(out, out_dtype, A, a_dtype, W, bias, M, N, K, st);
     case VB200_EPI_BIAS_GELU: return launch_gemm_dtype<VB200_EPI_BIAS_GELU>(out, out_dtype, A, a_dtype, W, bias, M, N, K, st);
     case VB200_EPI_BIAS_RESIDUAL:
-      if (residual != static_cast<const float*>(out))
-        VB_CHECK_CUDA(cudaMemcpyAsync(out, residual, static_cast<size_t>(M) * N * sizeof(float),
-                                      cudaMemcpyDeviceToDevice, st));
+      if (residual != static_cast<const float*>(out)) {
+        VB_REQUIRE((reinterpret_cast<uintptr_t>(residual) & 15) == 0, "gemm: residual must be 16-byte aligned");
+        return launch_gemm<gemm::EPI_RESIDUAL_ROWS, float>(out, out_dtype, A, a_dtype, W, bias, M, N, K, st, residual);
+      }
       return launch_gemm<VB200_EPI_BIAS_RESIDUAL, float>(out, out_dtype, A, a_dtype, W, bias, M, N, K, st);
   }
   set_error("gemm: unknown epilogue %d", static_cast<int>(epi));
   return VB200_ERR_INVALID;
 }
+
+extern "C" int vb200_gemm_residual_rows(void* out, vb200_dtype out_dtype, const void* A, vb200_dtype a_dtype,
+                                        const void* W, const float* bias, const float* residual,
+                                        const int32_t* residual_rows, int32_t M, int32_t N, int32_t K,
+                                        vb200_stream_t stream) {
+  VB_REQUIRE(M >= 0 && N > 0 && K > 0, "gemm_residual_rows: bad sizes M=%d N=%d K=%d", M, N, K);
+  VB_REQUIRE(a_dtype == VB200_BF16 || a_dtype == VB200_F16, "gemm_residual_rows: A and W must be bf16 or f16");
+  if (M == 0) return VB200_OK;
+  VB_REQUIRE(out && A && W && bias && residual, "gemm_residual_rows: null pointer");
+  VB_REQUIRE(residual != static_cast<const float*>(out), "gemm_residual_rows: residual must not alias out");
+  VB_REQUIRE(K % 8 == 0, "gemm_residual_rows: K=%d must be a multiple of 8", K);
+  VB_REQUIRE(N % 8 == 0, "gemm_residual_rows: N=%d must be a multiple of 8", N);
+  VB_REQUIRE((reinterpret_cast<uintptr_t>(out) & 15) == 0 && (reinterpret_cast<uintptr_t>(residual) & 15) == 0,
+             "gemm_residual_rows: out and residual must be 16-byte aligned");
+  return launch_gemm_dtype<gemm::EPI_RESIDUAL_ROWS>(out, out_dtype, A, a_dtype, W, bias, M, N, K,
+                                                    static_cast<cudaStream_t>(stream), residual, residual_rows);
+}
diff --git a/tts-with-diffusion-model_b200/vall_e/b200/engine.py b/tts-with-diffusion-model_b200/vall_e/b200/engine.py
--- a/tts-with-diffusion-model_b200/vall_e/b200/engine.py
+++ b/tts-with-diffusion-model_b200/vall_e/b200/engine.py
@@ -207,7 +207,9 @@
                        level_utt, w.K, levels_in)
         scale = 64 ** -0.5
         gemm, attn_flops = self._gemm, sum(4 * T * T * w.d for T in lay.rows)
-        for ly in w.layers:
+        all_rows = hidden_out is not None or sv or self.attn_variant != "tmem"
+        body = w.layers if all_rows else w.layers[:-1]
+        for ly in body:
             self._norm(ws.h, ws.x, ly["norm_attn"], level_utt, lay)
             gemm(ws.qkv, ws.h, ly["w_qkv"], epi=L.EPI_NONE)
             ev = self._prof_begin()
@@ -220,13 +222,36 @@
             gemm(ws.x, ws.ff, ly["w_ff2"], ly["b_ff2"], residual=ws.x, epi=L.EPI_BIAS_RESIDUAL)
             if hidden_out is not None:
                 hidden_out.append(ws.x.clone())
-        L.gather_rows_bf16(ws.head_in, ws.x, lay.resp_row_index)
-        self.launches += 1 + 7 * len(w.layers) + 1
+        if all_rows:
+            L.gather_rows_bf16(ws.head_in, ws.x, lay.resp_row_index)
+            self.launches += 1 + 7 * len(w.layers) + 1
+        else:
+            self._last_layer_resp_rows(lay, ws, level_utt, scale)
+            self.launches += 1 + 7 * len(w.layers)
         if not head:
             return ws.head_in
         gemm(ws.logits, ws.head_in, w.w_cls, w.b_cls, epi=L.EPI_BIAS)
         self.launches += 1
         return ws.logits
+
+    def _last_layer_resp_rows(self, lay, ws, level_utt, scale):
+        w, ly, Mr, d = self.w, self.w.layers[-1], lay.M_resp, self.w.d
+        self._norm(ws.h, ws.x, ly["norm_attn"], level_utt, lay)
+        self._gemm(ws.qkv, ws.h, ly["w_qkv"], epi=L.EPI_NONE)
+        att, h, ff = ws.att[:Mr], ws.h[:Mr], ws.ff[:Mr]
+        ev = self._prof_begin()
+        L.flash_attn_resp_rows(att, ws.qkv, lay.cu_rows, lay.utt, max(lay.t_resp), w.n_heads, scale)
+        self._prof_end(ev, "attn", sum(4 * T * Tr * d for T, Tr in zip(lay.rows, lay.t_resp)))
+        x_c = ws.qkv.view(-1)[:2 * Mr * d].view(torch.float32).view(Mr, d)
+        self._gemm_rows(x_c, att, ly["w_out"], ly["b_out"], ws.x, lay.resp_row_index)
+        self._norm(h, x_c, ly["norm_ffn"], level_utt, lay, lay.resp_row_utt)
+        self._gemm(ff, h, ly["w_ff1"], ly["b_ff1"], epi=L.EPI_BIAS_GELU)
+        self._gemm_rows(ws.head_in, ff, ly["w_ff2"], ly["b_ff2"], x_c)
+
+    def _gemm_rows(self, out, A, W, bias, residual, rows=None):
+        ev = self._prof_begin()
+        L.gemm_residual_rows(out, A, W, bias, residual, rows)
+        self._prof_end(ev, "gemm", 2 * A.shape[0] * A.shape[1] * W.shape[0])
 
     def _gemm(self, out, A, W, bias=None, residual=None, epi=L.EPI_NONE):
         ev = self._prof_begin()
@@ -247,10 +272,10 @@
         end.record()
         self.profile.append((kind, flops, ev, end))
 
-    def _norm(self, out, x, params, level_utt, lay):
+    def _norm(self, out, x, params, level_utt, lay, row_utt=None):
         ev = self._prof_begin()
         if self.w.norm_type == "adaln":
-            L.adaln(out, x, params, level_utt, lay.row_utt)
+            L.adaln(out, x, params, level_utt, lay.row_utt if row_utt is None else row_utt)
         else:
             L.layernorm(out, x, params[0], params[1])
         self._prof_end(ev, "norm", x.numel() * 6)
diff --git a/tts-with-diffusion-model_b200/vall_e/b200/lib.py b/tts-with-diffusion-model_b200/vall_e/b200/lib.py
--- a/tts-with-diffusion-model_b200/vall_e/b200/lib.py
+++ b/tts-with-diffusion-model_b200/vall_e/b200/lib.py
@@ -31,8 +31,10 @@
     "vb200_layernorm": ([_p, C.c_int] + [_p] * 3 + [_i32, _i32, _f, _p], C.c_int),
     "vb200_gather_rows_bf16": ([_p, C.c_int, _p, _p, _i32, _i32, _p], C.c_int),
     "vb200_gemm_bf16": ([_p, C.c_int, _p, C.c_int, _p, _p, _p, _i32, _i32, _i32, C.c_int, _p], C.c_int),
+    "vb200_gemm_residual_rows": ([_p, C.c_int, _p, C.c_int, _p, _p, _p, _p, _i32, _i32, _i32, _p], C.c_int),
     "vb200_gemm_bf16_simt": ([_p, C.c_int, _p, C.c_int, _p, _p, _p, _i32, _i32, _i32, C.c_int, _p], C.c_int),
     "vb200_flash_attn_varlen": ([_p, _p, _p, _i32, _i32, _i32, _i32, _f, _p], C.c_int),
+    "vb200_flash_attn_resp_rows": ([_p, _p, _p, _p, _i32, _i32, _i32, _i32, _f, _p], C.c_int),
     "vb200_attn_varlen_simt": ([_p, _p, _p, _i32, _i32, _i32, _i32, _f, _p], C.c_int),
     "vb200_q_sample": ([_p] * 6 + [_i32, _i32, _i32, C.c_int, _p], C.c_int),
     "vb200_q_sample_dense": ([_p] * 6 + [_i32, _i32, _i32, _p], C.c_int),
@@ -163,6 +165,26 @@
               stream()), "vb200_gemm_bf16")
 
 
+def gemm_residual_rows(out, A, W, bias, residual, rows=None):
+    M, K = A.shape
+    N = W.shape[0]
+    assert W.shape[1] == K and tuple(out.shape) == (M, N) and residual.shape[1] == N, (A.shape, W.shape, out.shape)
+    assert A.dtype in (torch.bfloat16, torch.float16) and W.dtype == A.dtype, (A.dtype, W.dtype)
+    assert residual.dtype == torch.float32 and (rows is None or (rows.dtype == torch.int32 and rows.numel() == M))
+    if rows is None:
+        assert residual.shape[0] >= M
+    _check(load().vb200_gemm_residual_rows(ptr(out), dtype_code(out.dtype), ptr(A), act_code(A), ptr(W), ptr(bias),
+                                           ptr(residual), ptr(rows), M, N, K, stream()), "vb200_gemm_residual_rows")
+
+
+def flash_attn_resp_rows(out, qkv, cu_rows, utt, max_T_resp, n_heads, scale):
+    M = qkv.shape[0]
+    B = cu_rows.numel() - 1
+    assert utt.shape == (B, U_STRIDE) and utt.dtype == torch.int32
+    _check(load().vb200_flash_attn_resp_rows(ptr(out), ptr(qkv), ptr(cu_rows), ptr(utt), B, max_T_resp, M, n_heads,
+                                             scale, stream()), "vb200_flash_attn_resp_rows")
+
+
 def flash_attn_varlen(out, qkv, cu_rows, max_T, n_heads, scale, variant="tmem"):
     M = qkv.shape[0]
     B = cu_rows.numel() - 1
```

After: 327,600 (median of 6 runs). 1.02x the previous value.
